# lambdaclass/lambda_elliptic_curves

Hardware: AMD Instinct MI355X
Metric: NTT elems/sec (Stark252 radix-2, 2^24, forward, bit-exact vs CPU: see 'bit_exact') [+ MSM G1 point-adds/sec under 'msm'] (higher is better)
Workload: dtype u32x8 (256-bit Montgomery, 32-bit limbs)

## Files before the change

### lambda_elliptic_curves_amd/csrc/field.cuh

```cuda
#pragma once
#include <stdint.h>

#if defined(__HIPCC__)
#include <hip/hip_runtime.h>
#define LW_HD __host__ __device__ __forceinline__
#else
#define LW_HD inline
#endif

namespace lw {

struct Stark252 {
    static constexpr int N = 8;
    static constexpr bool LAZY = true;
    static constexpr uint32_t INV = 0xffffffffu;
    static constexpr uint32_t TWO_ADICITY = 192;
    LW_HD static constexpr uint32_t p(int i) {
        constexpr uint32_t t[N] = {0x00000001u, 0x00000000u, 0x00000000u, 0x00000000u, 0x00000000u, 0x00000000u, 0x00000011u, 0x08000000u};
        return t[i];
    }
    LW_HD static constexpr uint32_t one(int i) {
        constexpr uint32_t t[N] = {0xffffffe1u, 0xffffffffu, 0xffffffffu, 0xffffffffu, 0xffffffffu, 0xffffffffu, 0xfffffdf0u, 0x07ffffffu};
        return t[i];
    }
    LW_HD static constexpr uint32_t r2(int i) {
        constexpr uint32_t t[N] = {0x7e000401u, 0xfffffd73u, 0x330fffffu, 0x00000001u, 0xff6f8000u, 0xffffffffu, 0x5e008810u, 0x07ffd4abu};
        return t[i];
    }
    LW_HD static constexpr uint32_t root(int i) {
        constexpr uint32_t t[N] = {0x42f8ef94u, 0x6070024fu, 0xe11a6161u, 0xad187148u, 0x9c8b0fa5u, 0x3f046451u, 0x87529cfau, 0x005282dbu};
        return t[i];
    }
};
struct Fr381 {
    static constexpr int N = 8;
    static constexpr bool LAZY = false;
    static constexpr uint32_t INV = 0xffffffffu;
    static constexpr uint32_t TWO_ADICITY = 32;
    LW_HD static constexpr uint32_t p(int i) {
        constexpr uint32_t t[N] = {0x00000001u, 0xffffffffu, 0xfffe5bfeu, 0x53bda402u, 0x09a1d805u, 0x3339d808u, 0x299d7d48u, 0x73eda753u};
        return t[i];
    }
    LW_HD static constexpr uint32_t one(int i) {
        constexpr uint32_t t[N] = {0xfffffffeu, 0x00000001u, 0x00034802u, 0x5884b7fau, 0xecbc4ff5u, 0x998c4fefu, 0xacc5056fu, 0x1824b159u};
        return t[i];
    }
    LW_HD static constexpr uint32_t r2(int i) {
        constexpr uint32_t t[N] = {0xf3f29c6du, 0xc999e990u, 0x87925c23u, 0x2b6cedcbu, 0x7254398fu, 0x05d31496u, 0x9f59ff11u, 0x0748d9d9u};
        return t[i];
    }
    LW_HD static constexpr uint32_t root(int i) {
        constexpr uint32_t t[N] = {0xbb30bbb7u, 0x54cc39d9u, 0xfa78eb2bu, 0xc5e433d6u, 0x349d9b3cu, 0x84dd396cu, 0xa08a499du, 0x2ab00961u};
        return t[i];
    }
};
struct Fp381 {
    static constexpr int N = 12;
    static constexpr uint32_t INV = 0xfffcfffdu;
    LW_HD static constexpr uint32_t p(int i) {
        constexpr uint32_t t[N] = {0xffffaaabu, 0xb9feffffu, 0xb153ffffu, 0x1eabfffeu, 0xf6b0f624u, 0x6730d2a0u, 0xf38512bfu, 0x64774b84u, 0x434bacd7u, 0x4b1ba7b6u, 0x397fe69au, 0x1a0111eau};
        return t[i];
    }
    LW_HD static constexpr uint32_t one(int i) {
        constexpr uint32_t t[N] = {0x0002fffdu, 0x76090000u, 0xc40c0002u, 0xebf4000bu, 0x53c758bau, 0x5f489857u, 0x70525745u, 0x77ce5853u, 0xa256ec6du, 0x5c071a97u, 0xfa80e493u, 0x15f65ec3u};
        return t[i];
    }
    LW_HD static constexpr uint32_t r2(int i) {
        constexpr uint32_t t[N] = {0x1c341746u, 0xf4df1f34u, 0x09d104f1u, 0x0a76e6a6u, 0x4c95b6d5u, 0x8de5476cu, 0x939d83c0u, 0x67eb88a9u, 0xb519952du, 0x9a793e85u, 0x92cae3aau, 0x11988fe5u};
        return t[i];
    }
};
struct Fp254 {
    static constexpr int N = 8;
    static constexpr uint32_t INV = 0xe4866389u;
    LW_HD static constexpr uint32_t p(int i) {
        constexpr uint32_t t[N] = {0xd87cfd47u, 0x3c208c16u, 0x6871ca8du, 0x97816a91u, 0x8181585du, 0xb85045b6u, 0xe131a029u, 0x30644e72u};
        return t[i];
    }
    LW_HD static constexpr uint32_t one(int i) {
        constexpr uint32_t t[N] = {0xc58f0d9du, 0xd35d438du, 0xf5c70b3du, 0x0a78eb28u, 0x7879462cu, 0x666ea36fu, 0x9a07df2fu, 0x0e0a77c1u};
        return t[i];
    }
    LW_HD static constexpr uint32_t r2(int i) {
        constexpr uint32_t t[N] = {0x538afa89u, 0xf32cfc5bu, 0xd44501fbu, 0xb5e71911u, 0x0a417ff6u, 0x47ab1effu, 0xcab8351fu, 0x06d89f71u};
        return t[i];
    }
};

struct Fr254 {
    static constexpr int N = 8;
    static constexpr uint32_t INV = 0xefffffffu;
    static constexpr bool LAZY = false;
    LW_HD static constexpr uint32_t p(int i) {
        constexpr uint32_t t[N] = {0xf0000001u, 0x43e1f593u, 0x79b97091u, 0x2833e848u, 0x8181585du, 0xb85045b6u, 0xe131a029u, 0x30644e72u};
        return t[i];
    }
    LW_HD static constexpr uint32_t one(int i) {
        constexpr uint32_t t[N] = {0x4ffffffbu, 0xac96341cu, 0x9f60cd29u, 0x36fc7695u, 0x7879462eu, 0x666ea36fu, 0x9a07df2fu, 0x0e0a77c1u};
        return t[i];
    }
    LW_HD static constexpr uint32_t r2(int i) {
        constexpr uint32_t t[N] = {0xae216da7u, 0x1bb8e645u, 0xe35c59e3u, 0x53fe3ab1u, 0x53bb8085u, 0x8c49833du, 0x7f4e44a5u, 0x0216d0b1u};
        return t[i];
    }
};

template <class F>
struct Fe {
    static constexpr int N = F::N;
    uint32_t v[F::N];

    LW_HD static Fe zero() {
        Fe r;
#pragma unroll
        for (int i = 0; i < N; i++) r.v[i] = 0;
        return r;
    }
    LW_HD static Fe one() {
        Fe r;
#pragma unroll
        for (int i = 0; i < N; i++) r.v[i] = F::one(i);
        return r;
    }
    LW_HD static Fe r2() {
        Fe r;
#pragma unroll
        for (int i = 0; i < N; i++) r.v[i] = F::r2(i);
        return r;
    }
    LW_HD bool is_zero() const {
        uint32_t o = 0;
#pragma unroll
        for (int i = 0; i < N; i++) o |= v[i];
        return o == 0;
    }
    LW_HD bool operator==(const Fe &b) const {
        uint32_t o = 0;
#pragma unroll
        for (int i = 0; i < N; i++) o |= v[i] ^ b.v[i];
        return o == 0;
    }
    LW_HD bool operator!=(const Fe &b) const { return !(*this == b); }
};

#if defined(__HIP_DEVICE_COMPILE__)
__device__ __forceinline__ uint32_t lw_k(uint32_t x) {
    asm("" : "+s"(x));
    return x;
}
#else
inline uint32_t lw_k(uint32_t x) { return x; }
#endif
#if defined(__clang__)
#define LW_ADDC(a, b, c) __builtin_addc((a), (b), (c), &(c))
#define LW_SUBC(a, b, c) __builtin_subc((a), (b), (c), &(c))
#else
static inline uint32_t lw_addc_portable(uint32_t a, uint32_t b, unsigned &c) {
    const uint64_t t = (uint64_t)a + b + c;
    c = (unsigned)(t >> 32);
    return (uint32_t)t;
}
static inline uint32_t lw_subc_portable(uint32_t a, uint32_t b, unsigned &c) {
    const uint64_t t = (uint64_t)a - b - c;
    c = (unsigned)((t >> 32) & 1);
    return (uint32_t)t;
}
#define LW_ADDC(a, b, c) lw_addc_portable((a), (b), (c))
#define LW_SUBC(a, b, c) lw_subc_portable((a), (b), (c))
#endif
template <int N>
LW_HD uint32_t limbs_add(uint32_t (&r)[N], const uint32_t (&a)[N], const uint32_t (&b)[N]) {
    unsigned c = 0;
#pragma unroll
    for (int i = 0; i < N; i++) r[i] = LW_ADDC(a[i], b[i], c);
    return c;
}
template <int N>
LW_HD uint32_t limbs_sub(uint32_t (&r)[N], const uint32_t (&a)[N], const uint32_t (&b)[N]) {
    unsigned c = 0;
#pragma unroll
    for (int i = 0; i < N; i++) r[i] = LW_SUBC(a[i], b[i], c);
    return c;
}
template <class F, int LOGK>
LW_HD constexpr uint32_t kp_limb(int i) {
    if (LOGK == 0) return F::p(i);
    return (F::p(i) << LOGK) | (i > 0 ? (F::p(i - 1) >> (32 - LOGK)) : 0u);
}
template <class F, int LOGK>
LW_HD void limbs_kp(uint32_t (&k)[F::N]) {
#pragma unroll
    for (int i = 0; i < F::N; i++) k[i] = lw_k(kp_limb<F, LOGK>(i));
}
template <class F>
LW_HD void limbs_p_masked(uint32_t (&k)[F::N], uint32_t mask) {
#pragma unroll
    for (int i = 0; i < F::N; i++) k[i] = F::p(i) == 0 ? lw_k(0u) : (lw_k(F::p(i)) & mask);
}

template <class F>
LW_HD Fe<F> reduce_once(const Fe<F> &a) {
    constexpr int N = F::N;
    uint32_t pk[N];
    limbs_kp<F, 0>(pk);
    Fe<F> d;
    const uint32_t borrow = limbs_sub<N>(d.v, a.v, pk);
    Fe<F> r;
#pragma unroll
    for (int i = 0; i < N; i++) r.v[i] = borrow ? a.v[i] : d.v[i];
    return r;
}

template <class F>
LW_HD Fe<F> fe_add(const Fe<F> &a, const Fe<F> &b) {
    Fe<F> s;
    limbs_add<F::N>(s.v, a.v, b.v);
    return reduce_once<F>(s);
}

template <class F>
LW_HD Fe<F> fe_sub(const Fe<F> &a, const Fe<F> &b) {
    constexpr int N = F::N;
    Fe<F> d;
    const uint32_t borrow = limbs_sub<N>(d.v, a.v, b.v);
    uint32_t pm[N];
    limbs_p_masked<F>(pm, 0u - borrow);
    Fe<F> r;
    limbs_add<N>(r.v, d.v, pm);
    return r;
}

template <class F>
LW_HD Fe<F> fe_neg(const Fe<F> &a) {
    constexpr int N = F::N;
    uint32_t nz = 0;
#pragma unroll
    for (int i = 0; i < N; i++) nz |= a.v[i];
    uint32_t pk[N];
    limbs_kp<F, 0>(pk);
    Fe<F> r;
    limbs_sub<N>(r.v, pk, a.v);
#pragma unroll
    for (int i = 0; i < N; i++) r.v[i] = nz ? r.v[i] : 0u;
    return r;
}

template <class F>
LW_HD Fe<F> fe_dbl(const Fe<F> &a) { return fe_add<F>(a, a); }

template <class F>
LW_HD Fe<F> fe_mul_portable(const Fe<F> &a, const Fe<F> &b) {
    constexpr int N = F::N;
    uint32_t t[N];
#pragma unroll
    for (int i = 0; i < N; i++) t[i] = 0;
#pragma unroll
    for (int i = 0; i < N; i++) {
        uint64_t c = 0;
#pragma unroll
        for (int j = 0; j < N; j++) {
            c += (uint64_t)a.v[j] * b.v[i] + t[j];
            t[j] = (uint32_t)c;
            c >>= 32;
        }
        uint32_t tN = (uint32_t)c;
        uint32_t m = t[0] * F::INV;
        c = ((uint64_t)m * F::p(0) + t[0]) >> 32;
#pragma unroll
        for (int j = 1; j < N; j++) {
            c += (uint64_t)m * F::p(j) + t[j];
            t[j - 1] = (uint32_t)c;
            c >>= 32;
        }
        c += tN;
        t[N - 1] = (uint32_t)c;
    }
    Fe<F> r;
#pragma unroll
    for (int i = 0; i < N; i++) r.v[i] = t[i];
    return reduce_once<F>(r);
}

#if !defined(__HIP_DEVICE_COMPILE__) && defined(__SIZEOF_INT128__)
#define LW_HOST_MUL64 1
template <class F>
inline Fe<F> fe_mul_host64(const Fe<F> &a, const Fe<F> &b) {
    constexpr int N = F::N, M = N / 2;
    static_assert(N % 2 == 0, "even number of 32-bit limbs");
    typedef unsigned __int128 u128;
    uint64_t A[M], B[M], P[M], t[M + 2];
    for (int i = 0; i < M; i++) {
        A[i] = (uint64_t)a.v[2 * i] | ((uint64_t)a.v[2 * i + 1] << 32);
        B[i] = (uint64_t)b.v[2 * i] | ((uint64_t)b.v[2 * i + 1] << 32);
        P[i] = (uint64_t)F::p(2 * i) | ((uint64_t)F::p(2 * i + 1) << 32);
    }
    for (int i = 0; i < M + 2; i++) t[i] = 0;
    uint64_t z = (uint64_t)(0u - F::INV);
    z *= 2 - P[0] * z;
    const uint64_t inv = 0 - z;
    for (int i = 0; i < M; i++) {
        u128 c = 0;
        for (int j = 0; j < M; j++) {
            c += (u128)A[j] * B[i] + t[j];
            t[j] = (uint64_t)c;
            c >>= 64;
        }
        c += t[M];
        t[M] = (uint64_t)c;
        t[M + 1] = (uint64_t)(c >> 64);
        const uint64_t m = t[0] * inv;
        c = ((u128)m * P[0] + t[0]) >> 64;
        for (int j = 1; j < M; j++) {
            c += (u128)m * P[j] + t[j];
            t[j - 1] = (uint64_t)c;
            c >>= 64;
        }
        c += t[M];
        t[M - 1] = (uint64_t)c;
        t[M] = t[M + 1] + (uint64_t)(c >> 64);
    }
    Fe<F> r;
    for (int i = 0; i < M; i++) {
        r.v[2 * i] = (uint32_t)t[i];
        r.v[2 * i + 1] = (uint32_t)(t[i] >> 32);
    }
    return reduce_once<F>(r);
}
#endif

#if defined(__HIP_DEVICE_COMPILE__)
#define LW_MAC_V(A, B) "v_mad_u64_u32 %0, vcc, " A ", " B ", %0\n\tv_addc_co_u32_e32 %1, vcc, 0, %1, vcc\n\t"

__device__ __forceinline__ void mac96_x1(uint64_t &lo, uint32_t &hi, uint32_t a0, uint32_t b0) {
    asm(LW_MAC_V("%2", "%3") : "+v"(lo), "+v"(hi) : "v"(a0), "v"(b0) : "vcc");
}
__device__ __forceinline__ void mac96_x2(uint64_t &lo, uint32_t &hi, uint32_t a0, uint32_t b0, uint32_t a1, uint32_t b1) {
    asm(LW_MAC_V("%2", "%3") LW_MAC_V("%4", "%5") : "+v"(lo), "+v"(hi) : "v"(a0), "v"(b0), "v"(a1), "v"(b1) : "vcc");
}
__device__ __forceinline__ void mac96_x4(uint64_t &lo, uint32_t &hi, uint32_t a0, uint32_t b0, uint32_t a1, uint32_t b1,
                                         uint32_t a2, uint32_t b2, uint32_t a3, uint32_t b3) {
    asm(LW_MAC_V("%2", "%3") LW_MAC_V("%4", "%5") LW_MAC_V("%6", "%7") LW_MAC_V("%8", "%9")
        : "+v"(lo), "+v"(hi)
        : "v"(a0), "v"(b0), "v"(a1), "v"(b1), "v"(a2), "v"(b2), "v"(a3), "v"(b3)
        : "vcc");
}
#define LW_MAC_FIRST(A, B, INIT) "v_mad_u64_u32 %0, vcc, " A ", " B ", " INIT "\n\tv_addc_co_u32_e64 %1, vcc, 0, 0, vcc\n\t"
template <uint32_t C>
__device__ __forceinline__ void mac96_c1(uint64_t &lo, uint32_t &hi, uint32_t m0) {
    if constexpr (C == 0) {
    } else if constexpr (C <= 64) {
        asm(LW_MAC_V("%2", "%3") : "+v"(lo), "+v"(hi) : "v"(m0), "n"(C) : "vcc");
    } else {
        asm(LW_MAC_V("%2", "%3") : "+v"(lo), "+v"(hi) : "v"(m0), "s"(C) : "vcc");
    }
}
template <uint32_t C0, uint32_t C1, uint32_t C2, uint32_t C3>
__device__ __forceinline__ void mac96_s4(uint64_t &lo, uint32_t &hi, uint32_t m0, uint32_t m1, uint32_t m2, uint32_t m3) {
    asm(LW_MAC_V("%2", "%3") LW_MAC_V("%4", "%5") LW_MAC_V("%6", "%7") LW_MAC_V("%8", "%9")
        : "+v"(lo), "+v"(hi)
        : "v"(m0), "s"(C0), "v"(m1), "s"(C1), "v"(m2), "s"(C2), "v"(m3), "s"(C3)
        : "vcc");
}

template <class F, int K, int I, int IEND>
__device__ __forceinline__ void col_ab(uint64_t &lo, uint32_t &hi, const Fe<F> &a, const Fe<F> &b) {
    if constexpr (I + 4 <= IEND) {
        mac96_x4(lo, hi, a.v[I], b.v[K - I], a.v[I + 1], b.v[K - I - 1], a.v[I + 2], b.v[K - I - 2], a.v[I + 3], b.v[K - I - 3]);
        col_ab<F, K, I + 4, IEND>(lo, hi, a, b);
    } else if constexpr (I + 2 <= IEND) {
        mac96_x2(lo, hi, a.v[I], b.v[K - I], a.v[I + 1], b.v[K - I - 1]);
        col_ab<F, K, I + 2, IEND>(lo, hi, a, b);
    } else if constexpr (I + 1 <= IEND) {
        mac96_x1(lo, hi, a.v[I], b.v[K - I]);
    }
}
template <uint32_t C>
constexpr bool lw_is_literal() { return C > 64; }
template <class F, int K, int I, int IEND>
__device__ __forceinline__ void col_mp(uint64_t &lo, uint32_t &hi, const uint32_t (&m)[F::N]) {
    if constexpr (I + 4 <= IEND) {
        if constexpr (lw_is_literal<F::p(K - I)>() && lw_is_literal<F::p(K - I - 1)>() && lw_is_literal<F::p(K - I - 2)>() &&
                      lw_is_literal<F::p(K - I - 3)>()) {
            mac96_s4<F::p(K - I), F::p(K - I - 1), F::p(K - I - 2), F::p(K - I - 3)>(lo, hi, m[I], m[I + 1], m[I + 2], m[I + 3]);
            col_mp<F, K, I + 4, IEND>(lo, hi, m);
        } else {
            mac96_c1<F::p(K - I)>(lo, hi, m[I]);
            col_mp<F, K, I + 1, IEND>(lo, hi, m);
        }
    } else if constexpr (I + 1 <= IEND) {
        mac96_c1<F::p(K - I)>(lo, hi, m[I]);
        col_mp<F, K, I + 1, IEND>(lo, hi, m);
    }
}
template <class F>
struct lw_fused_columns {
    static constexpr bool value = false;
};
template <class F, int K, bool A_LT_P>
struct FusedCol;
#include "mac_chains.inc"

template <class F, int LO, int HI>
constexpr bool lw_all_literal() {
    for (int i = LO; i < HI; i++)
        if (F::p(i) <= 64) return false;
    return true;
}

template <class F, int P, int K>
__device__ __forceinline__ void fips_col(uint64_t init, const Fe<F> *const (&a)[P], const Fe<F> *const (&b)[P], uint32_t (&m)[F::N],
                                         uint32_t (&t)[F::N]) {
    constexpr int N = F::N;
    if constexpr (K == 2 * N - 1) {
        t[N - 1] = (uint32_t)init;
    } else {
        uint64_t lo;
        uint32_t hi;
        if constexpr (K < N) {
            col_ab_first_dispatch<F, K, 0, K + 1>(lo, hi, init, *a[0], *b[0]);
            if constexpr (P > 1) col_ab<F, K, 0, K + 1>(lo, hi, *a[1], *b[1]);
            if constexpr (P > 2) col_ab<F, K, 0, K + 1>(lo, hi, *a[2], *b[2]);
            if constexpr (P > 3) col_ab<F, K, 0, K + 1>(lo, hi, *a[3], *b[3]);
            if constexpr (K >= 1 && lw_all_literal<F, 1, K + 1>()) col_mp_dispatch<F, K, 0, K>(lo, hi, m);
            else col_mp<F, K, 0, K>(lo, hi, m);
            uint32_t mk;
            if constexpr (F::INV == 0xffffffffu) mk = 0u - (uint32_t)lo;
            else mk = (uint32_t)lo * F::INV;
            m[K] = mk;
            mac96_c1<F::p(0)>(lo, hi, mk);
        } else {
            col_ab_first_dispatch<F, K, K - N + 1, 2 * N - 1 - K>(lo, hi, init, *a[0], *b[0]);
            if constexpr (P > 1) col_ab<F, K, K - N + 1, N>(lo, hi, *a[1], *b[1]);
            if constexpr (P > 2) col_ab<F, K, K - N + 1, N>(lo, hi, *a[2], *b[2]);
            if constexpr (P > 3) col_ab<F, K, K - N + 1, N>(lo, hi, *a[3], *b[3]);
            if constexpr (lw_all_literal<F, K - N + 1, N>()) col_mp_dispatch<F, K, K - N + 1, 2 * N - 1 - K>(lo, hi, m);
            else col_mp<F, K, K - N + 1, N>(lo, hi, m);
            t[K - N] = (uint32_t)lo;
        }
        fips_col<F, P, K + 1>((lo >> 32) | ((uint64_t)hi << 32), a, b, m, t);
    }
}
__device__ __forceinline__ void lw_redc_unit(uint32_t &m, uint32_t &mid, uint32_t &top, uint32_t t, uint32_t w1, uint32_t w2) {
    asm("v_sub_co_u32_e32 %0, vcc, 0, %3\n\t"
        "v_addc_co_u32_e32 %1, vcc, 0, %4, vcc\n\t"
        "v_addc_co_u32_e32 %2, vcc, 0, %5, vcc"
        : "=&v"(m), "=&v"(mid), "=v"(top)
        : "v"(t), "v"(w1), "v"(w2)
        : "vcc");
}
__device__ __forceinline__ void lw_redc_unit0(uint32_t &m, uint32_t &mid, uint32_t &top, uint32_t t, uint32_t w1) {
    asm("v_sub_co_u32_e32 %0, vcc, 0, %3\n\t"
        "v_addc_co_u32_e32 %1, vcc, 0, %4, vcc\n\t"
        "v_addc_co_u32_e64 %2, vcc, 0, 0, vcc"
        : "=&v"(m), "=&v"(mid), "=v"(top)
        : "v"(t), "v"(w1)
        : "vcc");
}
template <class F, int K, bool A_LT_P>
__device__ __forceinline__ void fips_fused(uint64_t init, const Fe<F> &a, const Fe<F> &b, uint32_t (&m)[F::N], uint32_t (&t)[F::N]) {
    constexpr int N = F::N;
    static_assert(F::p(0) == 1u && F::INV == 0xffffffffu, "fused columns need a unit low limb of the modulus");
    if constexpr (K == 2 * N - 1) {
        t[N - 1] = (uint32_t)init;
    } else {
        uint64_t lo;
        uint32_t hi;
        FusedCol<F, K, A_LT_P>::run(lo, hi, init, a, b, m);
        if constexpr (K < N) {
            uint32_t mid, top;
            if constexpr (K == 0) lw_redc_unit0(m[0], mid, top, (uint32_t)lo, (uint32_t)(lo >> 32));
            else lw_redc_unit(m[K], mid, top, (uint32_t)lo, (uint32_t)(lo >> 32), hi);
            fips_fused<F, K + 1, A_LT_P>(((uint64_t)top << 32) | mid, a, b, m, t);
        } else {
            t[K - N] = (uint32_t)lo;
            fips_fused<F, K + 1, A_LT_P>((lo >> 32) | ((uint64_t)hi << 32), a, b, m, t);
        }
    }
}
template <class F, bool A_LT_P = false>
__device__ __forceinline__ void fips_product(const Fe<F> &a, const Fe<F> &b, uint32_t (&t)[F::N]) {
    uint32_t m[F::N];
    if constexpr (lw_fused_columns<F>::value) {
        fips_fused<F, 0, A_LT_P>(0ull, a, b, m, t);
    } else {
        const Fe<F> *const pa[1] = {&a}, *const pb[1] = {&b};
        fips_col<F, 1, 0>(0ull, pa, pb, m, t);
    }
}
template <class F>
__device__ __forceinline__ Fe<F> fe_mul_gfx9(const Fe<F> &a, const Fe<F> &b) {
    constexpr int N = F::N;
    uint32_t t[N];
    fips_product<F>(a, b, t);
    Fe<F> r;
#pragma unroll
    for (int i = 0; i < N; i++) r.v[i] = t[i];
    return reduce_once<F>(r);
}
#endif

template <class F>
LW_HD Fe<F> fe_mul(const Fe<F> &a, const Fe<F> &b) {
#if defined(__HIP_DEVICE_COMPILE__)
    return fe_mul_gfx9<F>(a, b);
#elif defined(LW_HOST_MUL64)
    return fe_mul_host64<F>(a, b);
#else
    return fe_mul_portable<F>(a, b);
#endif
}

template <class F>
LW_HD Fe<F> fe_sqr(const Fe<F> &a) { return fe_mul<F>(a, a); }

template <class F>
LW_HD Fe<F> fe_neg_raw(const Fe<F> &a) {
    uint32_t pk[F::N];
    limbs_kp<F, 0>(pk);
    Fe<F> r;
    limbs_sub<F::N>(r.v, pk, a.v);
    return r;
}
template <class F>
LW_HD Fe<F> fe_neg_raw_2p(const Fe<F> &a) {
    uint32_t pk[F::N];
    limbs_kp<F, 1>(pk);
    Fe<F> r;
    limbs_sub<F::N>(r.v, pk, a.v);
    return r;
}
template <class F, int P, int KSUM = P>
LW_HD Fe<F> fe_dot(const Fe<F> *const (&a)[P], const Fe<F> *const (&b)[P]) {
    static_assert(P >= 1 && P <= 4, "fe_dot: 1..4 products");
    static_assert(KSUM >= P, "fe_dot: KSUM counts every product at least once");
    static_assert((uint64_t)KSUM * ((uint64_t)F::p(F::N - 1) + 1) <= (1ull << 32), "fe_dot: sum of products would exceed 2p after reduction");
#if defined(__HIP_DEVICE_COMPILE__)
    constexpr int N = F::N;
    uint32_t m[N], t[N];
    fips_col<F, P, 0>(0ull, a, b, m, t);
    Fe<F> r;
#pragma unroll
    for (int i = 0; i < N; i++) r.v[i] = t[i];
    return reduce_once<F>(r);
#else
    static_assert(KSUM == P, "fe_dot: unreduced operands are a device-code feature");
    Fe<F> acc = fe_mul<F>(reduce_once<F>(*a[0]), *b[0]);
    for (int q = 1; q < P; q++) acc = fe_add<F>(acc, fe_mul<F>(reduce_once<F>(*a[q]), *b[q]));
    return acc;
#endif
}

template <class F, int LOGK>
LW_HD Fe<F> fe_cond_sub_kp(const Fe<F> &a) {
    constexpr int N = F::N;
    uint32_t kp[N];
    limbs_kp<F, LOGK>(kp);
    Fe<F> d;
    const uint32_t borrow = limbs_sub<N>(d.v, a.v, kp);
    Fe<F> r;
#pragma unroll
    for (int i = 0; i < N; i++) r.v[i] = borrow ? a.v[i] : d.v[i];
    return r;
}
LW_HD Fe<Stark252> fe_reduce_full(const Fe<Stark252> &x) {
    const uint32_t q = x.v[7] >> 27;
    const uint32_t z = lw_k(0u);
    const uint32_t sub[8] = {q, z, z, z, z, z, 17u * q, q << 27};
    Fe<Stark252> d;
    const uint32_t borrow = limbs_sub<8>(d.v, x.v, sub);
    uint32_t pm[8];
    limbs_p_masked<Stark252>(pm, 0u - borrow);
    Fe<Stark252> r;
    limbs_add<8>(r.v, d.v, pm);
    return r;
}
template <class F>
LW_HD Fe<F> fe_reduce_full(const Fe<F> &x) { return reduce_once<F>(x); }

template <class F>
LW_HD Fe<F> fe_add_raw(const Fe<F> &a, const Fe<F> &b) {
    Fe<F> s;
    limbs_add<F::N>(s.v, a.v, b.v);
    return s;
}
template <class F>
LW_HD Fe<F> fe_add2p_sub_raw(const Fe<F> &a, const Fe<F> &b) {
    constexpr int N = F::N;
    uint32_t kp[N];
    limbs_kp<F, 1>(kp);
    Fe<F> d, r;
    limbs_sub<N>(d.v, a.v, b.v);
    limbs_add<N>(r.v, d.v, kp);
    return r;
}
template <class F>
LW_HD Fe<F> fe_mul_lazy(const Fe<F> &a, const Fe<F> &b) {
#if defined(__HIP_DEVICE_COMPILE__)
    constexpr int N = F::N;
    uint32_t t[N];
    fips_product<F, true>(a, b, t);
    Fe<F> r;
#pragma unroll
    for (int i = 0; i < N; i++) r.v[i] = t[i];
    return r;
#else
    return fe_mul_portable<F>(a, b);
#endif
}

template <class F>
LW_HD Fe<F> fe_pow_u64(Fe<F> base, uint64_t e) {
    Fe<F> r = Fe<F>::one();
    while (e) {
        if (e & 1) r = fe_mul<F>(r, base);
        base = fe_sqr<F>(base);
        e >>= 1;
    }
    return r;
}

template <class F>
LW_HD Fe<F> fe_inv(const Fe<F> &a) {
    constexpr int N = F::N;
    uint32_t e[N];
    uint64_t borrow = 2;
#pragma unroll
    for (int i = 0; i < N; i++) {
        uint64_t t = (uint64_t)F::p(i) - borrow;
        e[i] = (uint32_t)t;
        borrow = (t >> 32) & 1;
    }
    Fe<F> r = Fe<F>::one();
    for (int i = N - 1; i >= 0; i--) {
        for (int bit = 31; bit >= 0; bit--) {
            r = fe_sqr<F>(r);
            if ((e[i] >> bit) & 1) r = fe_mul<F>(r, a);
        }
    }
    return r;
}

template <class F>
LW_HD constexpr int fe_modulus_bits() {
    int top = 0;
    for (int b = 0; b < 32; b++)
        if ((F::p(F::N - 1) >> b) & 1u) top = b + 1;
    return 32 * (F::N - 1) + top;
}
template <int N>
LW_HD uint32_t bingcd_update_ab(uint32_t (&x)[N], uint32_t (&y)[N], int32_t f, int32_t g, int32_t h, int32_t k) {
    int64_t cx = 0, cy = 0;
    uint32_t wx[N + 1], wy[N + 1];
#pragma unroll
    for (int i = 0; i < N; i++) {
        const int64_t zx = (int64_t)x[i] * f + (int64_t)y[i] * g + cx;
        const int64_t zy = (int64_t)x[i] * h + (int64_t)y[i] * k + cy;
        wx[i] = (uint32_t)zx;
        wy[i] = (uint32_t)zy;
        cx = zx >> 32;
        cy = zy >> 32;
    }
    wx[N] = (uint32_t)cx;
    wy[N] = (uint32_t)cy;
    const uint32_t nx = (uint32_t)((uint64_t)cx >> 63), ny = (uint32_t)((uint64_t)cy >> 63);
    uint32_t carx = nx, cary = ny;
#pragma unroll
    for (int i = 0; i < N; i++) {
        uint32_t rx = (wx[i] >> 30) | (wx[i + 1] << 2), ry = (wy[i] >> 30) | (wy[i + 1] << 2);
        rx ^= 0u - nx;
        ry ^= 0u - ny;
        const uint32_t sx = rx + carx, sy = ry + cary;
        carx = sx < rx ? 1u : 0u;
        cary = sy < ry ? 1u : 0u;
        x[i] = sx;
        y[i] = sy;
    }
    return nx | (ny << 1);
}
template <class F>
LW_HD void bingcd_update_uv(uint32_t (&u)[F::N], uint32_t (&v)[F::N], int32_t f, int32_t g, int32_t h, int32_t k) {
    constexpr int N = F::N;
    const uint32_t fu = ((uint32_t)(u[0] * (uint32_t)f + v[0] * (uint32_t)g) * F::INV) & 0x3fffffffu;
    const uint32_t fv = ((uint32_t)(u[0] * (uint32_t)h + v[0] * (uint32_t)k) * F::INV) & 0x3fffffffu;
    int64_t cu = 0, cv = 0;
    uint32_t wu[N + 1], wv[N + 1];
#pragma unroll
    for (int i = 0; i < N; i++) {
        const int64_t zu = (int64_t)u[i] * f + (int64_t)v[i] * g + (int64_t)((uint64_t)F::p(i) * fu) + cu;
        const int64_t zv = (int64_t)u[i] * h + (int64_t)v[i] * k + (int64_t)((uint64_t)F::p(i) * fv) + cv;
        wu[i] = (uint32_t)zu;
        wv[i] = (uint32_t)zv;
        cu = zu >> 32;
        cv = zv >> 32;
    }
    wu[N] = (uint32_t)cu;
    wv[N] = (uint32_t)cv;
    const uint32_t nu = (uint32_t)((uint64_t)cu >> 63), nv = (uint32_t)((uint64_t)cv >> 63);
    uint32_t ru[N], rv[N];
#pragma unroll
    for (int i = 0; i < N; i++) {
        ru[i] = (wu[i] >> 30) | (wu[i + 1] << 2);
        rv[i] = (wv[i] >> 30) | (wv[i + 1] << 2);
    }
    uint32_t pk[N], du[N], dv[N], su[N], sv[N];
#pragma unroll
    for (int i = 0; i < N; i++) pk[i] = F::p(i);
    const uint32_t bu = limbs_sub<N>(du, ru, pk), bv = limbs_sub<N>(dv, rv, pk);
    limbs_add<N>(su, ru, pk);
    limbs_add<N>(sv, rv, pk);
#pragma unroll
    for (int i = 0; i < N; i++) {
        u[i] = nu ? su[i] : (bu ? ru[i] : du[i]);
        v[i] = nv ? sv[i] : (bv ? rv[i] : dv[i]);
    }
}
template <class F>
LW_HD Fe<F> fe_inv_int_bingcd(const Fe<F> &y) {
    constexpr int N = F::N;
    constexpr int ROUNDS = (2 * fe_modulus_bits<F>()) / 29 + 2;
    uint32_t a[N], b[N], u[N], v[N];
#pragma unroll
    for (int i = 0; i < N; i++) {
        a[i] = y.v[i];
        b[i] = F::p(i);
        u[i] = i == 0 ? 1u : 0u;
        v[i] = 0u;
    }
#pragma nounroll
    for (int round = 0; round < ROUNDS; round++) {
        uint32_t a0 = 0, a1 = 0, b0 = 0, b1 = 0, c0 = 0xffffffffu, c1 = 0xffffffffu;
#pragma unroll
        for (int j = N - 1; j >= 0; j--) {
            const uint32_t aw = a[j], bw = b[j];
            a0 ^= (a0 ^ aw) & c0;
            a1 ^= (a1 ^ aw) & c1;
            b0 ^= (b0 ^ bw) & c0;
            b1 ^= (b1 ^ bw) & c1;
            c1 = c0;
            c0 &= ((aw | bw) == 0u) ? 0xffffffffu : 0u;
        }
        a1 |= a0 & c1;
        a0 &= ~c1;
        b1 |= b0 & c1;
        b0 &= ~c1;
        uint64_t a_hi = ((uint64_t)a0 << 32) | a1, b_hi = ((uint64_t)b0 << 32) | b1;
        uint32_t a_lo = a[0], b_lo = b[0];
        int32_t pa = 1, pb = 0, qa = 0, qb = 1;
#pragma unroll 2
        for (int i = 0; i < 30; i++) {
            const uint32_t r = a_hi > b_hi ? 1u : 0u;
            const uint32_t oa = (a_lo >> i) & 1u, ob = (b_lo >> i) & 1u;
            const uint32_t cAB = oa & ob & r, cBA = oa & ob & (r ^ 1u), cA = cAB | (oa ^ 1u);
            const uint32_t mAB = 0u - cAB, mBA = 0u - cBA, mA = 0u - cA;
            a_lo -= b_lo & mAB;
            a_hi -= b_hi & (uint64_t)(int64_t)(int32_t)mAB;
            pa -= qa & (int32_t)mAB;
            pb -= qb & (int32_t)mAB;
            b_lo -= a_lo & mBA;
            b_hi -= a_hi & (uint64_t)(int64_t)(int32_t)mBA;
            qa -= pa & (int32_t)mBA;
            qb -= pb & (int32_t)mBA;
            a_lo += a_lo & ~mA;
            pa += pa & (int32_t)~mA;
            pb += pb & (int32_t)~mA;
            a_hi = cA ? (a_hi >> 1) : a_hi;
            b_lo += b_lo & mA;
            qa += qa & (int32_t)mA;
            qb += qb & (int32_t)mA;
            b_hi = cA ? b_hi : (b_hi >> 1);
        }
        const uint32_t neg = bingcd_update_ab<N>(a, b, pa, pb, qa, qb);
        if (neg & 1u) { pa = -pa; pb = -pb; }
        if (neg & 2u) { qa = -qa; qb = -qb; }
        bingcd_update_uv<F>(u, v, pa, pb, qa, qb);
    }
    Fe<F> r;
    const bool zero = y.is_zero();
#pragma unroll
    for (int i = 0; i < N; i++) r.v[i] = zero ? 0u : (u[i] | v[i]);
    return r;
}
template <class F>
LW_HD Fe<F> fe_inv_fast(const Fe<F> &a) {
    const Fe<F> r3 = fe_mul<F>(Fe<F>::r2(), Fe<F>::r2());
    return fe_mul<F>(fe_inv_int_bingcd<F>(a), r3);
}

template <class F>
LW_HD Fe<F> fe_to_mont(const Fe<F> &a) { return fe_mul<F>(a, Fe<F>::r2()); }
template <class F>
LW_HD Fe<F> fe_from_mont(const Fe<F> &a) {
    Fe<F> o = Fe<F>::zero();
    o.v[0] = 1;
    return fe_mul<F>(a, o);
}
template <class F>
LW_HD Fe<F> fe_from_u64(uint64_t x) {
    Fe<F> o = Fe<F>::zero();
    o.v[0] = (uint32_t)x;
    o.v[1] = (uint32_t)(x >> 32);
    return fe_to_mont<F>(o);
}

template <class F>
LW_HD constexpr int mem_index(int k) { return 2 * (F::N / 2 - 1 - k / 2) + (k & 1); }

template <class F>
LW_HD Fe<F> fe_load(const void *ptr) {
    constexpr int N = F::N;
    const uint4 *q = reinterpret_cast<const uint4 *>(ptr);
    uint32_t m[N];
#pragma unroll
    for (int i = 0; i < N / 4; i++) {
        uint4 x = q[i];
        m[4 * i + 0] = x.x; m[4 * i + 1] = x.y; m[4 * i + 2] = x.z; m[4 * i + 3] = x.w;
    }
    Fe<F> r;
#pragma unroll
    for (int k = 0; k < N; k++) r.v[k] = m[mem_index<F>(k)];
    return r;
}
template <class F>
LW_HD void fe_store(void *ptr, const Fe<F> &a) {
    constexpr int N = F::N;
    uint32_t m[N];
#pragma unroll
    for (int k = 0; k < N; k++) m[mem_index<F>(k)] = a.v[k];
    uint4 *q = reinterpret_cast<uint4 *>(ptr);
#pragma unroll
    for (int i = 0; i < N / 4; i++) q[i] = make_uint4(m[4 * i], m[4 * i + 1], m[4 * i + 2], m[4 * i + 3]);
}

struct BabyBear {
    static constexpr uint32_t P = 2013265921u;
    static constexpr uint32_t MU = 0x88000001u;
    static constexpr uint32_t R2 = 0x45dddde3u;
    static constexpr uint32_t ONE = 0x0ffffffeu;
    static constexpr uint32_t TWO_ADICITY = 24;
    static constexpr uint32_t ROOT = 21;
};

LW_HD uint32_t bb_reduce(uint64_t x) {
    const uint32_t m = (uint32_t)x * (0u - BabyBear::MU);
    const uint32_t r = (uint32_t)((x + (uint64_t)m * BabyBear::P) >> 32);
    const uint32_t d = r - BabyBear::P;
    return d < r ? d : r;
}
LW_HD uint32_t bb_mul(uint32_t a, uint32_t b) { return bb_reduce((uint64_t)a * b); }
LW_HD uint32_t bb_add(uint32_t a, uint32_t b) {
    const uint32_t s = a + b, d = s - BabyBear::P;
    return d < s ? d : s;
}
LW_HD uint32_t bb_sub(uint32_t a, uint32_t b) {
    const uint32_t d = a - b, e = d + BabyBear::P;
    return e < d ? e : d;
}
LW_HD uint32_t bb_pow(uint32_t a, uint64_t e) {
    uint32_t r = BabyBear::ONE;
    while (e) {
        if (e & 1) r = bb_mul(r, a);
        a = bb_mul(a, a);
        e >>= 1;
    }
    return r;
}
LW_HD uint32_t bb_inv(uint32_t a) { return bb_pow(a, (uint64_t)BabyBear::P - 2); }
LW_HD uint32_t bb_from_r64(uint64_t w) { return bb_reduce(w); }
LW_HD uint64_t bb_to_r64(uint32_t v) { return (uint64_t)bb_mul(v, BabyBear::R2); }

}
```

### lambda_elliptic_curves_amd/csrc/mac_chains.inc

```

template <class F, int K, int I>
__device__ __forceinline__ void col_ab_first_n1(uint64_t &lo, uint32_t &hi, uint64_t init, const Fe<F> &a, const Fe<F> &b) {
    asm(LW_MAC_FIRST("%3", "%4", "%2")
        : "=v"(lo), "=v"(hi)
        : "v"(init), "v"(a.v[I + 0]), "v"(b.v[K - I - 0])
        : "vcc");
}

template <class F, int K, int I>
__device__ __forceinline__ void col_ab_first_n2(uint64_t &lo, uint32_t &hi, uint64_t init, const Fe<F> &a, const Fe<F> &b) {
    asm(LW_MAC_FIRST("%3", "%4", "%2") LW_MAC_V("%5", "%6")
        : "=&v"(lo), "=&v"(hi)
        : "v"(init), "v"(a.v[I + 0]), "v"(b.v[K - I - 0]), "v"(a.v[I + 1]), "v"(b.v[K - I - 1])
        : "vcc");
}

template <class F, int K, int I>
__device__ __forceinline__ void col_ab_first_n3(uint64_t &lo, uint32_t &hi, uint64_t init, const Fe<F> &a, const Fe<F> &b) {
    asm(LW_MAC_FIRST("%3", "%4", "%2") LW_MAC_V("%5", "%6") LW_MAC_V("%7", "%8")
        : "=&v"(lo), "=&v"(hi)
        : "v"(init), "v"(a.v[I + 0]), "v"(b.v[K - I - 0]), "v"(a.v[I + 1]), "v"(b.v[K - I - 1]), "v"(a.v[I + 2]), "v"(b.v[K - I - 2])
        : "vcc");
}

template <class F, int K, int I>
__device__ __forceinline__ void col_ab_first_n4(uint64_t &lo, uint32_t &hi, uint64_t init, const Fe<F> &a, const Fe<F> &b) {
    asm(LW_MAC_FIRST("%3", "%4", "%2") LW_MAC_V("%5", "%6") LW_MAC_V("%7", "%8") LW_MAC_V("%9", "%10")
        : "=&v"(lo), "=&v"(hi)
        : "v"(init), "v"(a.v[I + 0]), "v"(b.v[K - I - 0]), "v"(a.v[I + 1]), "v"(b.v[K - I - 1]), "v"(a.v[I + 2]), "v"(b.v[K - I - 2]), "v"(a.v[I + 3]), "v"(b.v[K - I - 3])
        : "vcc");
}

template <class F, int K, int I>
__device__ __forceinline__ void col_ab_first_n5(uint64_t &lo, uint32_t &hi, uint64_t init, const Fe<F> &a, const Fe<F> &b) {
    asm(LW_MAC_FIRST("%3", "%4", "%2") LW_MAC_V("%5", "%6") LW_MAC_V("%7", "%8") LW_MAC_V("%9", "%10") LW_MAC_V("%11", "%12")
        : "=&v"(lo), "=&v"(hi)
        : "v"(init), "v"(a.v[I + 0]), "v"(b.v[K - I - 0]), "v"(a.v[I + 1]), "v"(b.v[K - I - 1]), "v"(a.v[I + 2]), "v"(b.v[K - I - 2]), "v"(a.v[I + 3]), "v"(b.v[K - I - 3]), "v"(a.v[I + 4]), "v"(b.v[K - I - 4])
        : "vcc");
}

template <class F, int K, int I>
__device__ __forceinline__ void col_ab_first_n6(uint64_t &lo, uint32_t &hi, uint64_t init, const Fe<F> &a, const Fe<F> &b) {
    asm(LW_MAC_FIRST("%3", "%4", "%2") LW_MAC_V("%5", "%6") LW_MAC_V("%7", "%8") LW_MAC_V("%9", "%10") LW_MAC_V("%11", "%12") LW_MAC_V("%13", "%14")
        : "=&v"(lo), "=&v"(hi)
        : "v"(init), "v"(a.v[I + 0]), "v"(b.v[K - I - 0]), "v"(a.v[I + 1]), "v"(b.v[K - I - 1]), "v"(a.v[I + 2]), "v"(b.v[K - I - 2]), "v"(a.v[I + 3]), "v"(b.v[K - I - 3]), "v"(a.v[I + 4]), "v"(b.v[K - I - 4]), "v"(a.v[I + 5]), "v"(b.v[K - I - 5])
        : "vcc");
}

template <class F, int K, int I>
__device__ __forceinline__ void col_ab_first_n7(uint64_t &lo, uint32_t &hi, uint64_t init, const Fe<F> &a, const Fe<F> &b) {
    asm(LW_MAC_FIRST("%3", "%4", "%2") LW_MAC_V("%5", "%6") LW_MAC_V("%7", "%8") LW_MAC_V("%9", "%10") LW_MAC_V("%11", "%12") LW_MAC_V("%13", "%14") LW_MAC_V("%15", "%16")
        : "=&v"(lo), "=&v"(hi)
        : "v"(init), "v"(a.v[I + 0]), "v"(b.v[K - I - 0]), "v"(a.v[I + 1]), "v"(b.v[K - I - 1]), "v"(a.v[I + 2]), "v"(b.v[K - I - 2]), "v"(a.v[I + 3]), "v"(b.v[K - I - 3]), "v"(a.v[I + 4]), "v"(b.v[K - I - 4]), "v"(a.v[I + 5]), "v"(b.v[K - I - 5]), "v"(a.v[I + 6]), "v"(b.v[K - I - 6])
        : "vcc");
}

template <class F, int K, int I>
__device__ __forceinline__ void col_ab_first_n8(uint64_t &lo, uint32_t &hi, uint64_t init, const Fe<F> &a, const Fe<F> &b) {
    asm(LW_MAC_FIRST("%3", "%4", "%2") LW_MAC_V("%5", "%6") LW_MAC_V("%7", "%8") LW_MAC_V("%9", "%10") LW_MAC_V("%11", "%12") LW_MAC_V("%13", "%14") LW_MAC_V("%15", "%16") LW_MAC_V("%17", "%18")
        : "=&v"(lo), "=&v"(hi)
        : "v"(init), "v"(a.v[I + 0]), "v"(b.v[K - I - 0]), "v"(a.v[I + 1]), "v"(b.v[K - I - 1]), "v"(a.v[I + 2]), "v"(b.v[K - I - 2]), "v"(a.v[I + 3]), "v"(b.v[K - I - 3]), "v"(a.v[I + 4]), "v"(b.v[K - I - 4]), "v"(a.v[I + 5]), "v"(b.v[K - I - 5]), "v"(a.v[I + 6]), "v"(b.v[K - I - 6]), "v"(a.v[I + 7]), "v"(b.v[K - I - 7])
        : "vcc");
}

template <class F, int K, int I>
__device__ __forceinline__ void col_ab_first_n9(uint64_t &lo, uint32_t &hi, uint64_t init, const Fe<F> &a, const Fe<F> &b) {
    asm(LW_MAC_FIRST("%3", "%4", "%2") LW_MAC_V("%5", "%6") LW_MAC_V("%7", "%8") LW_MAC_V("%9", "%10") LW_MAC_V("%11", "%12") LW_MAC_V("%13", "%14") LW_MAC_V("%15", "%16") LW_MAC_V("%17", "%18") LW_MAC_V("%19", "%20")
        : "=&v"(lo), "=&v"(hi)
        : "v"(init), "v"(a.v[I + 0]), "v"(b.v[K - I - 0]), "v"(a.v[I + 1]), "v"(b.v[K - I - 1]), "v"(a.v[I + 2]), "v"(b.v[K - I - 2]), "v"(a.v[I + 3]), "v"(b.v[K - I - 3]), "v"(a.v[I + 4]), "v"(b.v[K - I - 4]), "v"(a.v[I + 5]), "v"(b.v[K - I - 5]), "v"(a.v[I + 6]), "v"(b.v[K - I - 6]), "v"(a.v[I + 7]), "v"(b.v[K - I - 7]), "v"(a.v[I + 8]), "v"(b.v[K - I - 8])
        : "vcc");
}

template <class F, int K, int I>
__device__ __forceinline__ void col_ab_first_n10(uint64_t &lo, uint32_t &hi, uint64_t init, const Fe<F> &a, const Fe<F> &b) {
    asm(LW_MAC_FIRST("%3", "%4", "%2") LW_MAC_V("%5", "%6") LW_MAC_V("%7", "%8") LW_MAC_V("%9", "%10") LW_MAC_V("%11", "%12") LW_MAC_V("%13", "%14") LW_MAC_V("%15", "%16") LW_MAC_V("%17", "%18") LW_MAC_V("%19", "%20") LW_MAC_V("%21", "%22")
        : "=&v"(lo), "=&v"(hi)
        : "v"(init), "v"(a.v[I + 0]), "v"(b.v[K - I - 0]), "v"(a.v[I + 1]), "v"(b.v[K - I - 1]), "v"(a.v[I + 2]), "v"(b.v[K - I - 2]), "v"(a.v[I + 3]), "v"(b.v[K - I - 3]), "v"(a.v[I + 4]), "v"(b.v[K - I - 4]), "v"(a.v[I + 5]), "v"(b.v[K - I - 5]), "v"(a.v[I + 6]), "v"(b.v[K - I - 6]), "v"(a.v[I + 7]), "v"(b.v[K - I - 7]), "v"(a.v[I + 8]), "v"(b.v[K - I - 8]), "v"(a.v[I + 9]), "v"(b.v[K - I - 9])
        : "vcc");
}

template <class F, int K, int I>
__device__ __forceinline__ void col_ab_first_n11(uint64_t &lo, uint32_t &hi, uint64_t init, const Fe<F> &a, const Fe<F> &b) {
    asm(LW_MAC_FIRST("%3", "%4", "%2") LW_MAC_V("%5", "%6") LW_MAC_V("%7", "%8") LW_MAC_V("%9", "%10") LW_MAC_V("%11", "%12") LW_MAC_V("%13", "%14") LW_MAC_V("%15", "%16") LW_MAC_V("%17", "%18") LW_MAC_V("%19", "%20") LW_MAC_V("%21", "%22") LW_MAC_V("%23", "%24")
        : "=&v"(lo), "=&v"(hi)
        : "v"(init), "v"(a.v[I + 0]), "v"(b.v[K - I - 0]), "v"(a.v[I + 1]), "v"(b.v[K - I - 1]), "v"(a.v[I + 2]), "v"(b.v[K - I - 2]), "v"(a.v[I + 3]), "v"(b.v[K - I - 3]), "v"(a.v[I + 4]), "v"(b.v[K - I - 4]), "v"(a.v[I + 5]), "v"(b.v[K - I - 5]), "v"(a.v[I + 6]), "v"(b.v[K - I - 6]), "v"(a.v[I + 7]), "v"(b.v[K - I - 7]), "v"(a.v[I + 8]), "v"(b.v[K - I - 8]), "v"(a.v[I + 9]), "v"(b.v[K - I - 9]), "v"(a.v[I + 10]), "v"(b.v[K - I - 10])
        : "vcc");
}

template <class F, int K, int I>
__device__ __forceinline__ void col_ab_first_n12(uint64_t &lo, uint32_t &hi, uint64_t init, const Fe<F> &a, const Fe<F> &b) {
    asm(LW_MAC_FIRST("%3", "%4", "%2") LW_MAC_V("%5", "%6") LW_MAC_V("%7", "%8") LW_MAC_V("%9", "%10") LW_MAC_V("%11", "%12") LW_MAC_V("%13", "%14") LW_MAC_V("%15", "%16") LW_MAC_V("%17", "%18") LW_MAC_V("%19", "%20") LW_MAC_V("%21", "%22") LW_MAC_V("%23", "%24") LW_MAC_V("%25", "%26")
        : "=&v"(lo), "=&v"(hi)
        : "v"(init), "v"(a.v[I + 0]), "v"(b.v[K - I - 0]), "v"(a.v[I + 1]), "v"(b.v[K - I - 1]), "v"(a.v[I + 2]), "v"(b.v[K - I - 2]), "v"(a.v[I + 3]), "v"(b.v[K - I - 3]), "v"(a.v[I + 4]), "v"(b.v[K - I - 4]), "v"(a.v[I + 5]), "v"(b.v[K - I - 5]), "v"(a.v[I + 6]), "v"(b.v[K - I - 6]), "v"(a.v[I + 7]), "v"(b.v[K - I - 7]), "v"(a.v[I + 8]), "v"(b.v[K - I - 8]), "v"(a.v[I + 9]), "v"(b.v[K - I - 9]), "v"(a.v[I + 10]), "v"(b.v[K - I - 10]), "v"(a.v[I + 11]), "v"(b.v[K - I - 11])
        : "vcc");
}

template <class F, int K, int I>
__device__ __forceinline__ void col_mp_n1(uint64_t &lo, uint32_t &hi, const uint32_t (&m)[F::N]) {
    asm(LW_MAC_V("%2", "%3")
        : "+v"(lo), "+v"(hi)
        : "v"(m[I + 0]), "s"(F::p(K - I - 0))
        : "vcc");
}

template <class F, int K, int I>
__device__ __forceinline__ void col_mp_n2(uint64_t &lo, uint32_t &hi, const uint32_t (&m)[F::N]) {
    asm(LW_MAC_V("%2", "%3") LW_MAC_V("%4", "%5")
        : "+v"(lo), "+v"(hi)
        : "v"(m[I + 0]), "s"(F::p(K - I - 0)), "v"(m[I + 1]), "s"(F::p(K - I - 1))
        : "vcc");
}

template <class F, int K, int I>
__device__ __forceinline__ void col_mp_n3(uint64_t &lo, uint32_t &hi, const uint32_t (&m)[F::N]) {
    asm(LW_MAC_V("%2", "%3") LW_MAC_V("%4", "%5") LW_MAC_V("%6", "%7")
        : "+v"(lo), "+v"(hi)
        : "v"(m[I + 0]), "s"(F::p(K - I - 0)), "v"(m[I + 1]), "s"(F::p(K - I - 1)), "v"(m[I + 2]), "s"(F::p(K - I - 2))
        : "vcc");
}

template <class F, int K, int I>
__device__ __forceinline__ void col_mp_n4(uint64_t &lo, uint32_t &hi, const uint32_t (&m)[F::N]) {
    asm(LW_MAC_V("%2", "%3") LW_MAC_V("%4", "%5") LW_MAC_V("%6", "%7") LW_MAC_V("%8", "%9")
        : "+v"(lo), "+v"(hi)
        : "v"(m[I + 0]), "s"(F::p(K - I - 0)), "v"(m[I + 1]), "s"(F::p(K - I - 1)), "v"(m[I + 2]), "s"(F::p(K - I - 2)), "v"(m[I + 3]), "s"(F::p(K - I - 3))
        : "vcc");
}

template <class F, int K, int I>
__device__ __forceinline__ void col_mp_n5(uint64_t &lo, uint32_t &hi, const uint32_t (&m)[F::N]) {
    asm(LW_MAC_V("%2", "%3") LW_MAC_V("%4", "%5") LW_MAC_V("%6", "%7") LW_MAC_V("%8", "%9") LW_MAC_V("%10", "%11")
        : "+v"(lo), "+v"(hi)
        : "v"(m[I + 0]), "s"(F::p(K - I - 0)), "v"(m[I + 1]), "s"(F::p(K - I - 1)), "v"(m[I + 2]), "s"(F::p(K - I - 2)), "v"(m[I + 3]), "s"(F::p(K - I - 3)), "v"(m[I + 4]), "s"(F::p(K - I - 4))
        : "vcc");
}

template <class F, int K, int I>
__device__ __forceinline__ void col_mp_n6(uint64_t &lo, uint32_t &hi, const uint32_t (&m)[F::N]) {
    asm(LW_MAC_V("%2", "%3") LW_MAC_V("%4", "%5") LW_MAC_V("%6", "%7") LW_MAC_V("%8", "%9") LW_MAC_V("%10", "%11") LW_MAC_V("%12", "%13")
        : "+v"(lo), "+v"(hi)
        : "v"(m[I + 0]), "s"(F::p(K - I - 0)), "v"(m[I + 1]), "s"(F::p(K - I - 1)), "v"(m[I + 2]), "s"(F::p(K - I - 2)), "v"(m[I + 3]), "s"(F::p(K - I - 3)), "v"(m[I + 4]), "s"(F::p(K - I - 4)), "v"(m[I + 5]), "s"(F::p(K - I - 5))
        : "vcc");
}

template <class F, int K, int I>
__device__ __forceinline__ void col_mp_n7(uint64_t &lo, uint32_t &hi, const uint32_t (&m)[F::N]) {
    asm(LW_MAC_V("%2", "%3") LW_MAC_V("%4", "%5") LW_MAC_V("%6", "%7") LW_MAC_V("%8", "%9") LW_MAC_V("%10", "%11") LW_MAC_V("%12", "%13") LW_MAC_V("%14", "%15")
        : "+v"(lo), "+v"(hi)
        : "v"(m[I + 0]), "s"(F::p(K - I - 0)), "v"(m[I + 1]), "s"(F::p(K - I - 1)), "v"(m[I + 2]), "s"(F::p(K - I - 2)), "v"(m[I + 3]), "s"(F::p(K - I - 3)), "v"(m[I + 4]), "s"(F::p(K - I - 4)), "v"(m[I + 5]), "s"(F::p(K - I - 5)), "v"(m[I + 6]), "s"(F::p(K - I - 6))
        : "vcc");
}

template <class F, int K, int I>
__device__ __forceinline__ void col_mp_n8(uint64_t &lo, uint32_t &hi, const uint32_t (&m)[F::N]) {
    asm(LW_MAC_V("%2", "%3") LW_MAC_V("%4", "%5") LW_MAC_V("%6", "%7") LW_MAC_V("%8", "%9") LW_MAC_V("%10", "%11") LW_MAC_V("%12", "%13") LW_MAC_V("%14", "%15") LW_MAC_V("%16", "%17")
        : "+v"(lo), "+v"(hi)
        : "v"(m[I + 0]), "s"(F::p(K - I - 0)), "v"(m[I + 1]), "s"(F::p(K - I - 1)), "v"(m[I + 2]), "s"(F::p(K - I - 2)), "v"(m[I + 3]), "s"(F::p(K - I - 3)), "v"(m[I + 4]), "s"(F::p(K - I - 4)), "v"(m[I + 5]), "s"(F::p(K - I - 5)), "v"(m[I + 6]), "s"(F::p(K - I - 6)), "v"(m[I + 7]), "s"(F::p(K - I - 7))
        : "vcc");
}

template <class F, int K, int I>
__device__ __forceinline__ void col_mp_n9(uint64_t &lo, uint32_t &hi, const uint32_t (&m)[F::N]) {
    asm(LW_MAC_V("%2", "%3") LW_MAC_V("%4", "%5") LW_MAC_V("%6", "%7") LW_MAC_V("%8", "%9") LW_MAC_V("%10", "%11") LW_MAC_V("%12", "%13") LW_MAC_V("%14", "%15") LW_MAC_V("%16", "%17") LW_MAC_V("%18", "%19")
        : "+v"(lo), "+v"(hi)
        : "v"(m[I + 0]), "s"(F::p(K - I - 0)), "v"(m[I + 1]), "s"(F::p(K - I - 1)), "v"(m[I + 2]), "s"(F::p(K - I - 2)), "v"(m[I + 3]), "s"(F::p(K - I - 3)), "v"(m[I + 4]), "s"(F::p(K - I - 4)), "v"(m[I + 5]), "s"(F::p(K - I - 5)), "v"(m[I + 6]), "s"(F::p(K - I - 6)), "v"(m[I + 7]), "s"(F::p(K - I - 7)), "v"(m[I + 8]), "s"(F::p(K - I - 8))
        : "vcc");
}

template <class F, int K, int I>
__device__ __forceinline__ void col_mp_n10(uint64_t &lo, uint32_t &hi, const uint32_t (&m)[F::N]) {
    asm(LW_MAC_V("%2", "%3") LW_MAC_V("%4", "%5") LW_MAC_V("%6", "%7") LW_MAC_V("%8", "%9") LW_MAC_V("%10", "%11") LW_MAC_V("%12", "%13") LW_MAC_V("%14", "%15") LW_MAC_V("%16", "%17") LW_MAC_V("%18", "%19") LW_MAC_V("%20", "%21")
        : "+v"(lo), "+v"(hi)
        : "v"(m[I + 0]), "s"(F::p(K - I - 0)), "v"(m[I + 1]), "s"(F::p(K - I - 1)), "v"(m[I + 2]), "s"(F::p(K - I - 2)), "v"(m[I + 3]), "s"(F::p(K - I - 3)), "v"(m[I + 4]), "s"(F::p(K - I - 4)), "v"(m[I + 5]), "s"(F::p(K - I - 5)), "v"(m[I + 6]), "s"(F::p(K - I - 6)), "v"(m[I + 7]), "s"(F::p(K - I - 7)), "v"(m[I + 8]), "s"(F::p(K - I - 8)), "v"(m[I + 9]), "s"(F::p(K - I - 9))
        : "vcc");
}

template <class F, int K, int I>
__device__ __forceinline__ void col_mp_n11(uint64_t &lo, uint32_t &hi, const uint32_t (&m)[F::N]) {
    asm(LW_MAC_V("%2", "%3") LW_MAC_V("%4", "%5") LW_MAC_V("%6", "%7") LW_MAC_V("%8", "%9") LW_MAC_V("%10", "%11") LW_MAC_V("%12", "%13") LW_MAC_V("%14", "%15") LW_MAC_V("%16", "%17") LW_MAC_V("%18", "%19") LW_MAC_V("%20", "%21") LW_MAC_V("%22", "%23")
        : "+v"(lo), "+v"(hi)
        : "v"(m[I + 0]), "s"(F::p(K - I - 0)), "v"(m[I + 1]), "s"(F::p(K - I - 1)), "v"(m[I + 2]), "s"(F::p(K - I - 2)), "v"(m[I + 3]), "s"(F::p(K - I - 3)), "v"(m[I + 4]), "s"(F::p(K - I - 4)), "v"(m[I + 5]), "s"(F::p(K - I - 5)), "v"(m[I + 6]), "s"(F::p(K - I - 6)), "v"(m[I + 7]), "s"(F::p(K - I - 7)), "v"(m[I + 8]), "s"(F::p(K - I - 8)), "v"(m[I + 9]), "s"(F::p(K - I - 9)), "v"(m[I + 10]), "s"(F::p(K - I - 10))
        : "vcc");
}

template <class F, int K, int I, int CNT>
__device__ __forceinline__ void col_ab_first_dispatch(uint64_t &lo, uint32_t &hi, uint64_t init, const Fe<F> &a, const Fe<F> &b) {
    if constexpr (CNT == 1) col_ab_first_n1<F, K, I>(lo, hi, init, a, b);
    else if constexpr (CNT == 2) col_ab_first_n2<F, K, I>(lo, hi, init, a, b);
    else if constexpr (CNT == 3) col_ab_first_n3<F, K, I>(lo, hi, init, a, b);
    else if constexpr (CNT == 4) col_ab_first_n4<F, K, I>(lo, hi, init, a, b);
    else if constexpr (CNT == 5) col_ab_first_n5<F, K, I>(lo, hi, init, a, b);
    else if constexpr (CNT == 6) col_ab_first_n6<F, K, I>(lo, hi, init, a, b);
    else if constexpr (CNT == 7) col_ab_first_n7<F, K, I>(lo, hi, init, a, b);
    else if constexpr (CNT == 8) col_ab_first_n8<F, K, I>(lo, hi, init, a, b);
    else if constexpr (CNT == 9) col_ab_first_n9<F, K, I>(lo, hi, init, a, b);
    else if constexpr (CNT == 10) col_ab_first_n10<F, K, I>(lo, hi, init, a, b);
    else if constexpr (CNT == 11) col_ab_first_n11<F, K, I>(lo, hi, init, a, b);
    else if constexpr (CNT == 12) col_ab_first_n12<F, K, I>(lo, hi, init, a, b);
    else static_assert(CNT >= 1 && CNT <= 12, "unsupported MAC count");
}

template <class F, int K, int I, int CNT>
__device__ __forceinline__ void col_mp_dispatch(uint64_t &lo, uint32_t &hi, const uint32_t (&m)[F::N]) {
    if constexpr (CNT == 1) col_mp_n1<F, K, I>(lo, hi, m);
    else if constexpr (CNT == 2) col_mp_n2<F, K, I>(lo, hi, m);
    else if constexpr (CNT == 3) col_mp_n3<F, K, I>(lo, hi, m);
    else if constexpr (CNT == 4) col_mp_n4<F, K, I>(lo, hi, m);
    else if constexpr (CNT == 5) col_mp_n5<F, K, I>(lo, hi, m);
    else if constexpr (CNT == 6) col_mp_n6<F, K, I>(lo, hi, m);
    else if constexpr (CNT == 7) col_mp_n7<F, K, I>(lo, hi, m);
    else if constexpr (CNT == 8) col_mp_n8<F, K, I>(lo, hi, m);
    else if constexpr (CNT == 9) col_mp_n9<F, K, I>(lo, hi, m);
    else if constexpr (CNT == 10) col_mp_n10<F, K, I>(lo, hi, m);
    else if constexpr (CNT == 11) col_mp_n11<F, K, I>(lo, hi, m);
    else static_assert(CNT >= 1 && CNT <= 11, "unsupported MAC count");
}

static_assert(Stark252::N == 8 && Stark252::p(0) == 0x00000001u && Stark252::p(1) == 0x00000000u && Stark252::p(2) == 0x00000000u && Stark252::p(3) == 0x00000000u && Stark252::p(4) == 0x00000000u && Stark252::p(5) == 0x00000000u && Stark252::p(6) == 0x00000011u && Stark252::p(7) == 0x08000000u, "modulus changed: rerun tools/gen_mac_chains.py");
template <>
struct lw_fused_columns<Stark252> {
    static constexpr bool value = true;
};

template <>
struct FusedCol<Stark252, 0, false> {
    __device__ static __forceinline__ void run(uint64_t &lo, uint32_t &hi, uint64_t init, const Fe<Stark252> &a, const Fe<Stark252> &b, const uint32_t (&m)[8]) {
        asm("v_mad_u64_u32 %0, vcc, %1, %2, 0\n\t"
            : "=v"(lo)
            : "v"(a.v[0]), "v"(b.v[0])
            : "vcc");
        hi = 0;
    }
};

template <>
struct FusedCol<Stark252, 1, false> {
    __device__ static __forceinline__ void run(uint64_t &lo, uint32_t &hi, uint64_t init, const Fe<Stark252> &a, const Fe<Stark252> &b, const uint32_t (&m)[8]) {
        asm("v_mad_u64_u32 %0, vcc, %3, %4, %2\n\t"
            "v_mad_u64_u32 %0, vcc, %5, %6, %0\n\t"
            "v_addc_co_u32_e64 %1, vcc, 0, 0, vcc\n\t"
            : "=&v"(lo), "=&v"(hi)
            : "v"(init), "v"(a.v[0]), "v"(b.v[1]), "v"(a.v[1]), "v"(b.v[0])
            : "vcc");
    }
};

template <>
struct FusedCol<Stark252, 2, false> {
    __device__ static __forceinline__ void run(uint64_t &lo, uint32_t &hi, uint64_t init, const Fe<Stark252> &a, const Fe<Stark252> &b, const uint32_t (&m)[8]) {
        asm("v_mad_u64_u32 %0, vcc, %3, %4, %2\n\t"
            "v_mad_u64_u32 %0, vcc, %5, %6, %0\n\t"
            "v_addc_co_u32_e64 %1, vcc, 0, 0, vcc\n\t"
            "v_mad_u64_u32 %0, vcc, %7, %8, %0\n\t"
            "v_addc_co_u32_e32 %1, vcc, 0, %1, vcc\n\t"
            : "=&v"(lo), "=&v"(hi)
            : "v"(init), "v"(a.v[0]), "v"(b.v[2]), "v"(a.v[1]), "v"(b.v[1]), "v"(a.v[2]), "v"(b.v[0])
            : "vcc");
    }
};

template <>
struct FusedCol<Stark252, 3, false> {
    __device__ static __forceinline__ void run(uint64_t &lo, uint32_t &hi, uint64_t init, const Fe<Stark252> &a, const Fe<Stark252> &b, const uint32_t (&m)[8]) {
        asm("v_mad_u64_u32 %0, vcc, %3, %4, %2\n\t"
            "v_addc_co_u32_e64 %1, vcc, 0, 0, vcc\n\t"
            "v_mad_u64_u32 %0, vcc, %5, %6, %0\n\t"
            "v_addc_co_u32_e32 %1, vcc, 0, %1, vcc\n\t"
            "v_mad_u64_u32 %0, vcc, %7, %8, %0\n\t"
            "v_addc_co_u32_e32 %1, vcc, 0, %1, vcc\n\t"
            "v_mad_u64_u32 %0, vcc, %9, %10, %0\n\t"
            "v_addc_co_u32_e32 %1, vcc, 0, %1, vcc\n\t"
            : "=&v"(lo), "=&v"(hi)
            : "v"(init), "v"(a.v[0]), "v"(b.v[3]), "v"(a.v[1]), "v"(b.v[2]), "v"(a.v[2]), "v"(b.v[1]), "v"(a.v[3]), "v"(b.v[0])
            : "vcc");
    }
};

template <>
struct FusedCol<Stark252, 4, false> {
    __device__ static __forceinline__ void run(uint64_t &lo, uint32_t &hi, uint64_t init, const Fe<Stark252> &a, const Fe<Stark252> &b, const uint32_t (&m)[8]) {
        asm("v_mad_u64_u32 %0, vcc, %3, %4, %2\n\t"
            "v_addc_co_u32_e64 %1, vcc, 0, 0, vcc\n\t"
            "v_mad_u64_u32 %0, vcc, %5, %6, %0\n\t"
            "v_addc_co_u32_e32 %1, vcc, 0, %1, vcc\n\t"
            "v_mad_u64_u32 %0, vcc, %7, %8, %0\n\t"
            "v_addc_co_u32_e32 %1, vcc, 0, %1, vcc\n\t"
            "v_mad_u64_u32 %0, vcc, %9, %10, %0\n\t"
            "v_addc_co_u32_e32 %1, vcc, 0, %1, vcc\n\t"
            "v_mad_u64_u32 %0, vcc, %11, %12, %0\n\t"
            "v_addc_co_u32_e32 %1, vcc, 0, %1, vcc\n\t"
            : "=&v"(lo), "=&v"(hi)
            : "v"(init), "v"(a.v[0]), "v"(b.v[4]), "v"(a.v[1]), "v"(b.v[3]), "v"(a.v[2]), "v"(b.v[2]), "v"(a.v[3]), "v"(b.v[1]), "v"(a.v[4]), "v"(b.v[0])
            : "vcc");
    }
};

template <>
struct FusedCol<Stark252, 5, false> {
    __device__ static __forceinline__ void run(uint64_t &lo, uint32_t &hi, uint64_t init, const Fe<Stark252> &a, const Fe<Stark252> &b, const uint32_t (&m)[8]) {
        asm("v_mad_u64_u32 %0, vcc, %3, %4, %2\n\t"
            "v_addc_co_u32_e64 %1, vcc, 0, 0, vcc\n\t"
            "v_mad_u64_u32 %0, vcc, %5, %6, %0\n\t"
            "v_addc_co_u32_e32 %1, vcc, 0, %1, vcc\n\t"
            "v_mad_u64_u32 %0, vcc, %7, %8, %0\n\t"
            "v_addc_co_u32_e32 %1, vcc, 0, %1, vcc\n\t"
            "v_mad_u64_u32 %0, vcc, %9, %10, %0\n\t"
            "v_addc_co_u32_e32 %1, vcc, 0, %1, vcc\n\t"
            "v_mad_u64_u32 %0, vcc, %11, %12, %0\n\t"
            "v_addc_co_u32_e32 %1, vcc, 0, %1, vcc\n\t"
            "v_mad_u64_u32 %0, vcc, %13, %14, %0\n\t"
            "v_addc_co_u32_e32 %1, vcc, 0, %1, vcc\n\t"
            : "=&v"(lo), "=&v"(hi)
            : "v"(init), "v"(a.v[0]), "v"(b.v[5]), "v"(a.v[1]), "v"(b.v[4]), "v"(a.v[2]), "v"(b.v[3]), "v"(a.v[3]), "v"(b.v[2]), "v"(a.v[4]), "v"(b.v[1]), "v"(a.v[5]), "v"(b.v[0])
            : "vcc");
    }
};

template <>
struct FusedCol<Stark252, 6, false> {
    __device__ static __forceinline__ void run(uint64_t &lo, uint32_t &hi, uint64_t init, const Fe<Stark252> &a, const Fe<Stark252> &b, const uint32_t (&m)[8]) {
        asm("v_mad_u64_u32 %0, vcc, %3, 17, %2\n\t"
            "v_mad_u64_u32 %0, vcc, %4, %5, %0\n\t"
            "v_addc_co_u32_e64 %1, vcc, 0, 0, vcc\n\t"
            "v_mad_u64_u32 %0, vcc, %6, %7, %0\n\t"
            "v_addc_co_u32_e32 %1, vcc, 0, %1, vcc\n\t"
            "v_mad_u64_u32 %0, vcc, %8, %9, %0\n\t"
            "v_addc_co_u32_e32 %1, vcc, 0, %1, vcc\n\t"
            "v_mad_u64_u32 %0, vcc, %10, %11, %0\n\t"
            "v_addc_co_u32_e32 %1, vcc, 0, %1, vcc\n\t"
            "v_mad_u64_u32 %0, vcc, %12, %13, %0\n\t"
            "v_addc_co_u32_e32 %1, vcc, 0, %1, vcc\n\t"
            "v_mad_u64_u32 %0, vcc, %14, %15, %0\n\t"
            "v_addc_co_u32_e32 %1, vcc, 0, %1, vcc\n\t"
            "v_mad_u64_u32 %0, vcc, %16, %17, %0\n\t"
            "v_addc_co_u32_e32 %1, vcc, 0, %1, vcc\n\t"
            : "=&v"(lo), "=&v"(hi)
            : "v"(init), "v"(m[0]), "v"(a.v[0]), "v"(b.v[6]), "v"(a.v[1]), "v"(b.v[5]), "v"(a.v[2]), "v"(b.v[4]), "v"(a.v[3]), "v"(b.v[3]), "v"(a.v[4]), "v"(b.v[2]), "v"(a.v[5]), "v"(b.v[1]), "v"(a.v[6]), "v"(b.v[0])
            : "vcc");
    }
};

template <>
struct FusedCol<Stark252, 7, false> {
    __device__ static __forceinline__ void run(uint64_t &lo, uint32_t &hi, uint64_t init, const Fe<Stark252> &a, const Fe<Stark252> &b, const uint32_t (&m)[8]) {
        asm("v_mad_u64_u32 %0, vcc, %3, %4, %2\n\t"
            "v_mad_u64_u32 %0, vcc, %5, 17, %0\n\t"
            "v_mad_u64_u32 %0, vcc, %6, %7, %0\n\t"
            "v_addc_co_u32_e64 %1, vcc, 0, 0, vcc\n\t"
            "v_mad_u64_u32 %0, vcc, %8, %9, %0\n\t"
            "v_addc_co_u32_e32 %1, vcc, 0, %1, vcc\n\t"
            "v_mad_u64_u32 %0, vcc, %10, %11, %0\n\t"
            "v_addc_co_u32_e32 %1, vcc, 0, %1, vcc\n\t"
            "v_mad_u64_u32 %0, vcc, %12, %13, %0\n\t"
            "v_addc_co_u32_e32 %1, vcc, 0, %1, vcc\n\t"
            "v_mad_u64_u32 %0, vcc, %14, %15, %0\n\t"
            "v_addc_co_u32_e32 %1, vcc, 0, %1, vcc\n\t"
            "v_mad_u64_u32 %0, vcc, %16, %17, %0\n\t"
            "v_addc_co_u32_e32 %1, vcc, 0, %1, vcc\n\t"
            "v_mad_u64_u32 %0, vcc, %18, %19, %0\n\t"
            "v_addc_co_u32_e32 %1, vcc, 0, %1, vcc\n\t"
            "v_mad_u64_u32 %0, vcc, %20, %21, %0\n\t"
            "v_addc_co_u32_e32 %1, vcc, 0, %1, vcc\n\t"
            : "=&v"(lo), "=&v"(hi)
            : "v"(init), "v"(m[0]), "s"(Stark252::p(7)), "v"(m[1]), "v"(a.v[0]), "v"(b.v[7]), "v"(a.v[1]), "v"(b.v[6]), "v"(a.v[2]), "v"(b.v[5]), "v"(a.v[3]), "v"(b.v[4]), "v"(a.v[4]), "v"(b.v[3]), "v"(a.v[5]), "v"(b.v[2]), "v"(a.v[6]), "v"(b.v[1]), "v"(a.v[7]), "v"(b.v[0])
            : "vcc");
    }
};

template <>
struct FusedCol<Stark252, 8, false> {
    __device__ static __forceinline__ void run(uint64_t &lo, uint32_t &hi, uint64_t init, const Fe<Stark252> &a, const Fe<Stark252> &b, const uint32_t (&m)[8]) {
        asm("v_mad_u64_u32 %0, vcc, %3, %4, %2\n\t"
            "v_mad_u64_u32 %0, vcc, %5, 17, %0\n\t"
            "v_mad_u64_u32 %0, vcc, %6, %7, %0\n\t"
            "v_addc_co_u32_e64 %1, vcc, 0, 0, vcc\n\t"
            "v_mad_u64_u32 %0, vcc, %8, %9, %0\n\t"
            "v_addc_co_u32_e32 %1, vcc, 0, %1, vcc\n\t"
            "v_mad_u64_u32 %0, vcc, %10, %11, %0\n\t"
            "v_addc_co_u32_e32 %1, vcc, 0, %1, vcc\n\t"
            "v_mad_u64_u32 %0, vcc, %12, %13, %0\n\t"
            "v_addc_co_u32_e32 %1, vcc, 0, %1, vcc\n\t"
            "v_mad_u64_u32 %0, vcc, %14, %15, %0\n\t"
            "v_addc_co_u32_e32 %1, vcc, 0, %1, vcc\n\t"
            "v_mad_u64_u32 %0, vcc, %16, %17, %0\n\t"
            "v_addc_co_u32_e32 %1, vcc, 0, %1, vcc\n\t"
            "v_mad_u64_u32 %0, vcc, %18, %19, %0\n\t"
            "v_addc_co_u32_e32 %1, vcc, 0, %1, vcc\n\t"
            : "=&v"(lo), "=&v"(hi)
            : "v"(init), "v"(m[1]), "s"(Stark252::p(7)), "v"(m[2]), "v"(a.v[1]), "v"(b.v[7]), "v"(a.v[2]), "v"(b.v[6]), "v"(a.v[3]), "v"(b.v[5]), "v"(a.v[4]), "v"(b.v[4]), "v"(a.v[5]), "v"(b.v[3]), "v"(a.v[6]), "v"(b.v[2]), "v"(a.v[7]), "v"(b.v[1])
            : "vcc");
    }
};

template <>
struct FusedCol<Stark252, 9, false> {
    __device__ static __forceinline__ void run(uint64_t &lo, uint32_t &hi, uint64_t init, const Fe<Stark252> &a, const Fe<Stark252> &b, const uint32_t (&m)[8]) {
        asm("v_mad_u64_u32 %0, vcc, %3, %4, %2\n\t"
            "v_mad_u64_u32 %0, vcc, %5, 17, %0\n\t"
            "v_mad_u64_u32 %0, vcc, %6, %7, %0\n\t"
            "v_addc_co_u32_e64 %1, vcc, 0, 0, vcc\n\t"
            "v_mad_u64_u32 %0, vcc, %8, %9, %0\n\t"
            "v_addc_co_u32_e32 %1, vcc, 0, %1, vcc\n\t"
            "v_mad_u64_u32 %0, vcc, %10, %11, %0\n\t"
            "v_addc_co_u32_e32 %1, vcc, 0, %1, vcc\n\t"
            "v_mad_u64_u32 %0, vcc, %12, %13, %0\n\t"
            "v_addc_co_u32_e32 %1, vcc, 0, %1, vcc\n\t"
            "v_mad_u64_u32 %0, vcc, %14, %15, %0\n\t"
            "v_addc_co_u32_e32 %1, vcc, 0, %1, vcc\n\t"
            "v_mad_u64_u32 %0, vcc, %16, %17, %0\n\t"
            "v_addc_co_u32_e32 %1, vcc, 0, %1, vcc\n\t"
            : "=&v"(lo), "=&v"(hi)
            : "v"(init), "v"(m[2]), "s"(Stark252::p(7)), "v"(m[3]), "v"(a.v[2]), "v"(b.v[7]), "v"(a.v[3]), "v"(b.v[6]), "v"(a.v[4]), "v"(b.v[5]), "v"(a.v[5]), "v"(b.v[4]), "v"(a.v[6]), "v"(b.v[3]), "v"(a.v[7]), "v"(b.v[2])
            : "vcc");
    }
};

template <>
struct FusedCol<Stark252, 10, false> {
    __device__ static __forceinline__ void run(uint64_t &lo, uint32_t &hi, uint64_t init, const Fe<Stark252> &a, const Fe<Stark252> &b, const uint32_t (&m)[8]) {
        asm("v_mad_u64_u32 %0, vcc, %3, %4, %2\n\t"
            "v_mad_u64_u32 %0, vcc, %5, 17, %0\n\t"
            "v_mad_u64_u32 %0, vcc, %6, %7, %0\n\t"
            "v_addc_co_u32_e64 %1, vcc, 0, 0, vcc\n\t"
            "v_mad_u64_u32 %0, vcc, %8, %9, %0\n\t"
            "v_addc_co_u32_e32 %1, vcc, 0, %1, vcc\n\t"
            "v_mad_u64_u32 %0, vcc, %10, %11, %0\n\t"
            "v_addc_co_u32_e32 %1, vcc, 0, %1, vcc\n\t"
            "v_mad_u64_u32 %0, vcc, %12, %13, %0\n\t"
            "v_addc_co_u32_e32 %1, vcc, 0, %1, vcc\n\t"
            "v_mad_u64_u32 %0, vcc, %14, %15, %0\n\t"
            "v_addc_co_u32_e32 %1, vcc, 0, %1, vcc\n\t"
            : "=&v"(lo), "=&v"(hi)
            : "v"(init), "v"(m[3]), "s"(Stark252::p(7)), "v"(m[4]), "v"(a.v[3]), "v"(b.v[7]), "v"(a.v[4]), "v"(b.v[6]), "v"(a.v[5]), "v"(b.v[5]), "v"(a.v[6]), "v"(b.v[4]), "v"(a.v[7]), "v"(b.v[3])
            : "vcc");
    }
};

template <>
struct FusedCol<Stark252, 11, false> {
    __device__ static __forceinline__ void run(uint64_t &lo, uint32_t &hi, uint64_t init, const Fe<Stark252> &a, const Fe<Stark252> &b, const uint32_t (&m)[8]) {
        asm("v_mad_u64_u32 %0, vcc, %3, %4, %2\n\t"
            "v_mad_u64_u32 %0, vcc, %5, 17, %0\n\t"
            "v_mad_u64_u32 %0, vcc, %6, %7, %0\n\t"
            "v_addc_co_u32_e64 %1, vcc, 0, 0, vcc\n\t"
            "v_mad_u64_u32 %0, vcc, %8, %9, %0\n\t"
            "v_addc_co_u32_e32 %1, vcc, 0, %1, vcc\n\t"
            "v_mad_u64_u32 %0, vcc, %10, %11, %0\n\t"
            "v_addc_co_u32_e32 %1, vcc, 0, %1, vcc\n\t"
            "v_mad_u64_u32 %0, vcc, %12, %13, %0\n\t"
            "v_addc_co_u32_e32 %1, vcc, 0, %1, vcc\n\t"
            : "=&v"(lo), "=&v"(hi)
            : "v"(init), "v"(m[4]), "s"(Stark252::p(7)), "v"(m[5]), "v"(a.v[4]), "v"(b.v[7]), "v"(a.v[5]), "v"(b.v[6]), "v"(a.v[6]), "v"(b.v[5]), "v"(a.v[7]), "v"(b.v[4])
            : "vcc");
    }
};

template <>
struct FusedCol<Stark252, 12, false> {
    __device__ static __forceinline__ void run(uint64_t &lo, uint32_t &hi, uint64_t init, const Fe<Stark252> &a, const Fe<Stark252> &b, const uint32_t (&m)[8]) {
        asm("v_mad_u64_u32 %0, vcc, %3, %4, %2\n\t"
            "v_mad_u64_u32 %0, vcc, %5, 17, %0\n\t"
            "v_mad_u64_u32 %0, vcc, %6, %7, %0\n\t"
            "v_addc_co_u32_e64 %1, vcc, 0, 0, vcc\n\t"
            "v_mad_u64_u32 %0, vcc, %8, %9, %0\n\t"
            "v_addc_co_u32_e32 %1, vcc, 0, %1, vcc\n\t"
            "v_mad_u64_u32 %0, vcc, %10, %11, %0\n\t"
            "v_addc_co_u32_e32 %1, vcc, 0, %1, vcc\n\t"
            : "=&v"(lo), "=&v"(hi)
            : "v"(init), "v"(m[5]), "s"(Stark252::p(7)), "v"(m[6]), "v"(a.v[5]), "v"(b.v[7]), "v"(a.v[6]), "v"(b.v[6]), "v"(a.v[7]), "v"(b.v[5])
            : "vcc");
    }
};

template <>
struct FusedCol<Stark252, 13, false> {
    __device__ static __forceinline__ void run(uint64_t &lo, uint32_t &hi, uint64_t init, const Fe<Stark252> &a, const Fe<Stark252> &b, const uint32_t (&m)[8]) {
        asm("v_mad_u64_u32 %0, vcc, %3, %4, %2\n\t"
            "v_mad_u64_u32 %0, vcc, %5, 17, %0\n\t"
            "v_mad_u64_u32 %0, vcc, %6, %7, %0\n\t"
            "v_addc_co_u32_e64 %1, vcc, 0, 0, vcc\n\t"
            "v_mad_u64_u32 %0, vcc, %8, %9, %0\n\t"
            "v_addc_co_u32_e32 %1, vcc, 0, %1, vcc\n\t"
            : "=&v"(lo), "=&v"(hi)
            : "v"(init), "v"(m[6]), "s"(Stark252::p(7)), "v"(m[7]), "v"(a.v[6]), "v"(b.v[7]), "v"(a.v[7]), "v"(b.v[6])
            : "vcc");
    }
};

template <>
struct FusedCol<Stark252, 14, false> {
    __device__ static __forceinline__ void run(uint64_t &lo, uint32_t &hi, uint64_t init, const Fe<Stark252> &a, const Fe<Stark252> &b, const uint32_t (&m)[8]) {
        asm("v_mad_u64_u32 %0, vcc, %2, %3, %1\n\t"
            "v_mad_u64_u32 %0, vcc, %4, %5, %0\n\t"
            : "=&v"(lo)
            : "v"(init), "v"(m[7]), "s"(Stark252::p(7)), "v"(a.v[7]), "v"(b.v[7])
            : "vcc");
        hi = 0;
    }
};

template <>
struct FusedCol<Stark252, 0, true> : FusedCol<Stark252, 0, false> {};

template <>
struct FusedCol<Stark252, 1, true> : FusedCol<Stark252, 1, false> {};

template <>
struct FusedCol<Stark252, 2, true> : FusedCol<Stark252, 2, false> {};

template <>
struct FusedCol<Stark252, 3, true> : FusedCol<Stark252, 3, false> {};

template <>
struct FusedCol<Stark252, 4, true> : FusedCol<Stark252, 4, false> {};

template <>
struct FusedCol<Stark252, 5, true> : FusedCol<Stark252, 5, false> {};

template <>
struct FusedCol<Stark252, 6, true> : FusedCol<Stark252, 6, false> {};

template <>
struct FusedCol<Stark252, 7, true> {
    __device__ static __forceinline__ void run(uint64_t &lo, uint32_t &hi, uint64_t init, const Fe<Stark252> &a, const Fe<Stark252> &b, const uint32_t (&m)[8]) {
        asm("v_mad_u64_u32 %0, vcc, %3, %4, %2\n\t"
            "v_mad_u64_u32 %0, vcc, %5, 17, %0\n\t"
            "v_mad_u64_u32 %0, vcc, %6, %7, %0\n\t"
            "v_mad_u64_u32 %0, vcc, %8, %9, %0\n\t"
            "v_addc_co_u32_e64 %1, vcc, 0, 0, vcc\n\t"
            "v_mad_u64_u32 %0, vcc, %10, %11, %0\n\t"
            "v_addc_co_u32_e32 %1, vcc, 0, %1, vcc\n\t"
            "v_mad_u64_u32 %0, vcc, %12, %13, %0\n\t"
            "v_addc_co_u32_e32 %1, vcc, 0, %1, vcc\n\t"
            "v_mad_u64_u32 %0, vcc, %14, %15, %0\n\t"
            "v_addc_co_u32_e32 %1, vcc, 0, %1, vcc\n\t"
            "v_mad_u64_u32 %0, vcc, %16, %17, %0\n\t"
            "v_addc_co_u32_e32 %1, vcc, 0, %1, vcc\n\t"
            "v_mad_u64_u32 %0, vcc, %18, %19, %0\n\t"
            "v_addc_co_u32_e32 %1, vcc, 0, %1, vcc\n\t"
            "v_mad_u64_u32 %0, vcc, %20, %21, %0\n\t"
            "v_addc_co_u32_e32 %1, vcc, 0, %1, vcc\n\t"
            : "=&v"(lo), "=&v"(hi)
            : "v"(init), "v"(m[0]), "s"(Stark252::p(7)), "v"(m[1]), "v"(a.v[7]), "v"(b.v[0]), "v"(a.v[0]), "v"(b.v[7]), "v"(a.v[1]), "v"(b.v[6]), "v"(a.v[2]), "v"(b.v[5]), "v"(a.v[3]), "v"(b.v[4]), "v"(a.v[4]), "v"(b.v[3]), "v"(a.v[5]), "v"(b.v[2]), "v"(a.v[6]), "v"(b.v[1])
            : "vcc");
    }
};

template <>
struct FusedCol<Stark252, 8, true> {
    __device__ static __forceinline__ void run(uint64_t &lo, uint32_t &hi, uint64_t init, const Fe<Stark252> &a, const Fe<Stark252> &b, const uint32_t (&m)[8]) {
        asm("v_mad_u64_u32 %0, vcc, %3, %4, %2\n\t"
            "v_mad_u64_u32 %0, vcc, %5, 17, %0\n\t"
            "v_mad_u64_u32 %0, vcc, %6, %7, %0\n\t"
            "v_mad_u64_u32 %0, vcc, %8, %9, %0\n\t"
            "v_addc_co_u32_e64 %1, vcc, 0, 0, vcc\n\t"
            "v_mad_u64_u32 %0, vcc, %10, %11, %0\n\t"
            "v_addc_co_u32_e32 %1, vcc, 0, %1, vcc\n\t"
            "v_mad_u64_u32 %0, vcc, %12, %13, %0\n\t"
            "v_addc_co_u32_e32 %1, vcc, 0, %1, vcc\n\t"
            "v_mad_u64_u32 %0, vcc, %14, %15, %0\n\t"
            "v_addc_co_u32_e32 %1, vcc, 0, %1, vcc\n\t"
            "v_mad_u64_u32 %0, vcc, %16, %17, %0\n\t"
            "v_addc_co_u32_e32 %1, vcc, 0, %1, vcc\n\t"
            "v_mad_u64_u32 %0, vcc, %18, %19, %0\n\t"
            "v_addc_co_u32_e32 %1, vcc, 0, %1, vcc\n\t"
            : "=&v"(lo), "=&v"(hi)
            : "v"(init), "v"(m[1]), "s"(Stark252::p(7)), "v"(m[2]), "v"(a.v[7]), "v"(b.v[1]), "v"(a.v[1]), "v"(b.v[7]), "v"(a.v[2]), "v"(b.v[6]), "v"(a.v[3]), "v"(b.v[5]), "v"(a.v[4]), "v"(b.v[4]), "v"(a.v[5]), "v"(b.v[3]), "v"(a.v[6]), "v"(b.v[2])
            : "vcc");
    }
};

template <>
struct FusedCol<Stark252, 9, true> {
    __device__ static __forceinline__ void run(uint64_t &lo, uint32_t &hi, uint64_t init, const Fe<Stark252> &a, const Fe<Stark252> &b, const uint32_t (&m)[8]) {
        asm("v_mad_u64_u32 %0, vcc, %3, %4, %2\n\t"
            "v_mad_u64_u32 %0, vcc, %5, 17, %0\n\t"
            "v_mad_u64_u32 %0, vcc, %6, %7, %0\n\t"
            "v_mad_u64_u32 %0, vcc, %8, %9, %0\n\t"
            "v_addc_co_u32_e64 %1, vcc, 0, 0, vcc\n\t"
            "v_mad_u64_u32 %0, vcc, %10, %11, %0\n\t"
            "v_addc_co_u32_e32 %1, vcc, 0, %1, vcc\n\t"
            "v_mad_u64_u32 %0, vcc, %12, %13, %0\n\t"
            "v_addc_co_u32_e32 %1, vcc, 0, %1, vcc\n\t"
            "v_mad_u64_u32 %0, vcc, %14, %15, %0\n\t"
            "v_addc_co_u32_e32 %1, vcc, 0, %1, vcc\n\t"
            "v_mad_u64_u32 %0, vcc, %16, %17, %0\n\t"
            "v_addc_co_u32_e32 %1, vcc, 0, %1, vcc\n\t"
            : "=&v"(lo), "=&v"(hi)
            : "v"(init), "v"(m[2]), "s"(Stark252::p(7)), "v"(m[3]), "v"(a.v[7]), "v"(b.v[2]), "v"(a.v[2]), "v"(b.v[7]), "v"(a.v[3]), "v"(b.v[6]), "v"(a.v[4]), "v"(b.v[5]), "v"(a.v[5]), "v"(b.v[4]), "v"(a.v[6]), "v"(b.v[3])
            : "vcc");
    }
};

template <>
struct FusedCol<Stark252, 10, true> {
    __device__ static __forceinline__ void run(uint64_t &lo, uint32_t &hi, uint64_t init, const Fe<Stark252> &a, const Fe<Stark252> &b, const uint32_t (&m)[8]) {
        asm("v_mad_u64_u32 %0, vcc, %3, %4, %2\n\t"
            "v_mad_u64_u32 %0, vcc, %5, 17, %0\n\t"
            "v_mad_u64_u32 %0, vcc, %6, %7, %0\n\t"
            "v_mad_u64_u32 %0, vcc, %8, %9, %0\n\t"
            "v_addc_co_u32_e64 %1, vcc, 0, 0, vcc\n\t"
            "v_mad_u64_u32 %0, vcc, %10, %11, %0\n\t"
            "v_addc_co_u32_e32 %1, vcc, 0, %1, vcc\n\t"
            "v_mad_u64_u32 %0, vcc, %12, %13, %0\n\t"
            "v_addc_co_u32_e32 %1, vcc, 0, %1, vcc\n\t"
            "v_mad_u64_u32 %0, vcc, %14, %15, %0\n\t"
            "v_addc_co_u32_e32 %1, vcc, 0, %1, vcc\n\t"
            : "=&v"(lo), "=&v"(hi)
            : "v"(init), "v"(m[3]), "s"(Stark252::p(7)), "v"(m[4]), "v"(a.v[7]), "v"(b.v[3]), "v"(a.v[3]), "v"(b.v[7]), "v"(a.v[4]), "v"(b.v[6]), "v"(a.v[5]), "v"(b.v[5]), "v"(a.v[6]), "v"(b.v[4])
            : "vcc");
    }
};

template <>
struct FusedCol<Stark252, 11, true> {
    __device__ static __forceinline__ void run(uint64_t &lo, uint32_t &hi, uint64_t init, const Fe<Stark252> &a, const Fe<Stark252> &b, const uint32_t (&m)[8]) {
        asm("v_mad_u64_u32 %0, vcc, %3, %4, %2\n\t"
            "v_mad_u64_u32 %0, vcc, %5, 17, %0\n\t"
            "v_mad_u64_u32 %0, vcc, %6, %7, %0\n\t"
            "v_mad_u64_u32 %0, vcc, %8, %9, %0\n\t"
            "v_addc_co_u32_e64 %1, vcc, 0, 0, vcc\n\t"
            "v_mad_u64_u32 %0, vcc, %10, %11, %0\n\t"
            "v_addc_co_u32_e32 %1, vcc, 0, %1, vcc\n\t"
            "v_mad_u64_u32 %0, vcc, %12, %13, %0\n\t"
            "v_addc_co_u32_e32 %1, vcc, 0, %1, vcc\n\t"
            : "=&v"(lo), "=&v"(hi)
            : "v"(init), "v"(m[4]), "s"(Stark252::p(7)), "v"(m[5]), "v"(a.v[7]), "v"(b.v[4]), "v"(a.v[4]), "v"(b.v[7]), "v"(a.v[5]), "v"(b.v[6]), "v"(a.v[6]), "v"(b.v[5])
            : "vcc");
    }
};

template <>
struct FusedCol<Stark252, 12, true> {
    __device__ static __forceinline__ void run(uint64_t &lo, uint32_t &hi, uint64_t init, const Fe<Stark252> &a, const Fe<Stark252> &b, const uint32_t (&m)[8]) {
        asm("v_mad_u64_u32 %0, vcc, %3, %4, %2\n\t"
            "v_mad_u64_u32 %0, vcc, %5, 17, %0\n\t"
            "v_mad_u64_u32 %0, vcc, %6, %7, %0\n\t"
            "v_mad_u64_u32 %0, vcc, %8, %9, %0\n\t"
            "v_addc_co_u32_e64 %1, vcc, 0, 0, vcc\n\t"
            "v_mad_u64_u32 %0, vcc, %10, %11, %0\n\t"
            "v_addc_co_u32_e32 %1, vcc, 0, %1, vcc\n\t"
            : "=&v"(lo), "=&v"(hi)
            : "v"(init), "v"(m[5]), "s"(Stark252::p(7)), "v"(m[6]), "v"(a.v[7]), "v"(b.v[5]), "v"(a.v[5]), "v"(b.v[7]), "v"(a.v[6]), "v"(b.v[6])
            : "vcc");
    }
};

template <>
struct FusedCol<Stark252, 13, true> {
    __device__ static __forceinline__ void run(uint64_t &lo, uint32_t &hi, uint64_t init, const Fe<Stark252> &a, const Fe<Stark252> &b, const uint32_t (&m)[8]) {
        asm("v_mad_u64_u32 %0, vcc, %3, %4, %2\n\t"
            "v_mad_u64_u32 %0, vcc, %5, 17, %0\n\t"
            "v_mad_u64_u32 %0, vcc, %6, %7, %0\n\t"
            "v_mad_u64_u32 %0, vcc, %8, %9, %0\n\t"
            "v_addc_co_u32_e64 %1, vcc, 0, 0, vcc\n\t"
            : "=&v"(lo), "=&v"(hi)
            : "v"(init), "v"(m[6]), "s"(Stark252::p(7)), "v"(m[7]), "v"(a.v[7]), "v"(b.v[6]), "v"(a.v[6]), "v"(b.v[7])
            : "vcc");
    }
};

template <>
struct FusedCol<Stark252, 14, true> : FusedCol<Stark252, 14, false> {};
```

### lambda_elliptic_curves_amd/csrc/ntt_kernels.cuh

```cuda
#pragma once
#include "field.cuh"

namespace lw {

constexpr int NTT_TILE_LOG = 11;
constexpr int NTT_TILE = 1 << NTT_TILE_LOG;
constexpr int NTT_THREADS = 512;
constexpr int NTT_KMAX = 2;
constexpr int NTT_WG_PER_CU = (160 * 1024) / (NTT_TILE * 32 + 8192) > 8 ? 8 : (160 * 1024) / (NTT_TILE * 32 + 8192);
constexpr int NTT_WAVES_PER_SIMD = (NTT_WG_PER_CU * NTT_THREADS / 256) > 8 ? 8 : (NTT_WG_PER_CU * NTT_THREADS / 256) < 1 ? 1 : (NTT_WG_PER_CU * NTT_THREADS / 256);
constexpr int NTT_LTW = 256;

struct NttPassParams {
    const uint4 *in;
    uint4 *out;
    const uint4 *tw;
    uint64_t in_batch_stride;
    uint64_t out_batch_stride;
    uint32_t L;
    uint32_t s0;
    uint32_t r;
    uint32_t logC;
    uint32_t nsteps;
    uint32_t k[8];
    const uint4 *cos_lo, *cos_hi;
    uint32_t cos_hbits;
    uint32_t cos_in;
    uint32_t cos_out;
    uint64_t in_mask;
    uint32_t lazy_in;
    uint32_t wave_sync;
    uint32_t scale;
    uint32_t sc[8];
};

__device__ __forceinline__ uint32_t bitrev_bits(uint32_t x, uint32_t bits) {
    return bits ? (__brev(x) >> (32 - bits)) : 0u;
}

template <class F>
__device__ __forceinline__ Fe<F> tw_load(const uint4 *tw, uint64_t g) {
    uint4 a = tw[2 * g], b = tw[2 * g + 1];
    Fe<F> r;
    r.v[0] = a.x; r.v[1] = a.y; r.v[2] = a.z; r.v[3] = a.w;
    r.v[4] = b.x; r.v[5] = b.y; r.v[6] = b.z; r.v[7] = b.w;
    return r;
}
template <class F>
__device__ __forceinline__ void tw_store(uint4 *tw, uint64_t g, const Fe<F> &x) {
    tw[2 * g] = make_uint4(x.v[0], x.v[1], x.v[2], x.v[3]);
    tw[2 * g + 1] = make_uint4(x.v[4], x.v[5], x.v[6], x.v[7]);
}

template <class F>
__device__ __forceinline__ Fe<F> unpack_mem(uint4 q0, uint4 q1) {
    Fe<F> r;
    r.v[6] = q0.x; r.v[7] = q0.y; r.v[4] = q0.z; r.v[5] = q0.w;
    r.v[2] = q1.x; r.v[3] = q1.y; r.v[0] = q1.z; r.v[1] = q1.w;
    return r;
}
template <class F>
__device__ __forceinline__ void pack_mem(const Fe<F> &a, uint4 &q0, uint4 &q1) {
    q0 = make_uint4(a.v[6], a.v[7], a.v[4], a.v[5]);
    q1 = make_uint4(a.v[2], a.v[3], a.v[0], a.v[1]);
}

template <bool WL>
__device__ __forceinline__ uint32_t lds_slot(uint32_t m, uint32_t c, uint32_t r, uint32_t logC) {
    if (!WL) return (m << logC) | c;
    const uint32_t sw = r >= 4 ? ((5u * ((m >> 4) & 3u)) ^ ((c & 7u) << 1)) : 0u;
    return (c << r) | (m ^ sw);
}
__device__ __forceinline__ void lds_wave_sync() {
    __builtin_amdgcn_fence(__ATOMIC_RELEASE, "wavefront");
    __builtin_amdgcn_wave_barrier();
    __builtin_amdgcn_fence(__ATOMIC_ACQUIRE, "wavefront");
}

template <class F, int K, bool LAST, bool EXTRA, bool WL, int FX = 0>
__device__ __forceinline__ void ntt_item(const NttPassParams &p, uint4 (*lds)[NTT_TILE], uint4 (*ltw)[NTT_LTW], const uint4 *gin,
                                         uint4 *gout, uint32_t w, uint32_t step, uint32_t t0, uint64_t base, uint32_t lgS,
                                         uint32_t hi_uniform, uint32_t hi_low, bool last_step, bool stage_tw) {
    constexpr int E = 1 << K;
    const uint32_t r = FX ? (uint32_t)FX : p.r, logC = FX ? (uint32_t)(NTT_TILE_LOG - FX) : p.logC, L = p.L;
    const uint32_t sh = r - t0 - K;
    uint32_t c, mr;
    if ((LAST && step == 0) || (WL && (LAST || step > 0))) {
        mr = w & ((1u << (r - K)) - 1);
        c = w >> (r - K);
    } else {
        c = w & ((1u << logC) - 1);
        mr = w >> logC;
    }
    const uint32_t m_low = mr & ((1u << sh) - 1);
    const uint32_t m_high = mr >> sh;
    const uint32_t mbase = (m_high << (sh + K)) | m_low;
    uint32_t hi_c = hi_uniform;
    uint64_t gbase = base;
    if (LAST) {
        hi_c = (bitrev_bits(c, logC) << (L - r - logC)) | hi_low;
        gbase = (uint64_t)hi_c << r;
    }

    uint4 tq0, tq1;
    const uint32_t ti = threadIdx.x;
    if (!LAST && !WL && stage_tw && ti + 1 < (1u << r)) {
        const uint32_t t = 31 - __clz(ti + 1), xg = ti + 1 - (1u << t);
        const uint64_t g = ((uint64_t)hi_uniform << t) | xg;
        tq0 = p.tw[2 * g];
        tq1 = p.tw[2 * g + 1];
    }

    Fe<F> x[E];
    if (step == 0) {
#pragma unroll
        for (int j = 0; j < E; j++) {
            const uint32_t m = mbase | ((uint32_t)j << sh);
            const uint64_t g = (LAST ? (gbase + m) : (gbase + ((uint64_t)m << lgS) + c)) & p.in_mask;
            x[j] = unpack_mem<F>(gin[2 * g], gin[2 * g + 1]);
        }
        if (EXTRA && p.cos_in) {
#pragma unroll
            for (int j = 0; j < E; j++) {
                const uint32_t m = mbase | ((uint32_t)j << sh);
                const uint64_t e = (LAST ? (gbase + m) : (gbase + ((uint64_t)m << lgS) + c)) & p.in_mask;
                Fe<F> pw = fe_mul<F>(tw_load<F>(p.cos_lo, e & ((1ull << p.cos_hbits) - 1)), tw_load<F>(p.cos_hi, e >> p.cos_hbits));
                x[j] = fe_mul<F>(x[j], pw);
            }
        }
    } else {
#pragma unroll
        for (int j = 0; j < E; j++) {
            const uint32_t idx = lds_slot<WL>(mbase | ((uint32_t)j << sh), c, r, logC);
            x[j] = unpack_mem<F>(lds[0][idx], lds[1][idx ^ (WL ? 1u : 0u)]);
        }
    }

    if (!LAST && !WL && stage_tw) {
        if (ti + 1 < (1u << r)) {
            ltw[0][ti] = tq0;
            ltw[1][ti] = tq1;
        }
        __syncthreads();
    }

    if (F::LAZY && step == 0 && p.lazy_in) {
#pragma unroll
        for (int j = 0; j < E / 2; j++) x[j] = fe_reduce_full(x[j]);
    }

    auto fetch_tw = [&](int q) -> Fe<F> {
        const int u = 31 - __builtin_clz(q + 1), jt = q + 1 - (1 << u);
        Fe<F> tw;
        if (LAST || WL) {
            const uint64_t gt = ((uint64_t)hi_c << (t0 + u)) | ((uint64_t)m_high << u);
            tw = tw_load<F>(p.tw, gt | (uint32_t)jt);
        } else {
            const uint32_t li = (1u << (t0 + u)) - 1 + ((m_high << u) | (uint32_t)jt);
            uint4 a = ltw[0][li], b = ltw[1][li];
            tw.v[0] = a.x; tw.v[1] = a.y; tw.v[2] = a.z; tw.v[3] = a.w;
            tw.v[4] = b.x; tw.v[5] = b.y; tw.v[6] = b.z; tw.v[7] = b.w;
        }
        return tw;
    };
    Fe<F> tw_next = fetch_tw(0);
#pragma unroll
    for (int q = 0; q < E - 1; q++) {
        const int u = 31 - __builtin_clz(q + 1), jt = q + 1 - (1 << u);
        const int half = 1 << (K - 1 - u);
        const Fe<F> tw = tw_next;
        if (q + 1 < E - 1) tw_next = fetch_tw(q + 1);
        const bool unit = (jt == 0) && (hi_c == 0) && (m_high == 0);
#pragma unroll
        for (int jl = 0; jl < half; jl++) {
            const int j = (jt << (K - u)) | jl;
            if (F::LAZY) {
                Fe<F> wb = unit ? fe_reduce_full(x[j + half]) : fe_mul_lazy<F>(tw, x[j + half]);
                Fe<F> a = x[j];
                x[j] = fe_add_raw<F>(a, wb);
                x[j + half] = fe_add2p_sub_raw<F>(a, wb);
            } else {
                Fe<F> wb = unit ? x[j + half] : fe_mul<F>(tw, x[j + half]);
                Fe<F> a = x[j];
                x[j] = fe_add<F>(a, wb);
                x[j + half] = fe_sub<F>(a, wb);
            }
            __builtin_amdgcn_sched_barrier(0);
        }
    }

    if (EXTRA && LAST && last_step && p.cos_out) {
#pragma unroll
        for (int j = 0; j < E; j++) {
            const uint32_t m = mbase | ((uint32_t)j << sh);
            const uint64_t i_nat = ((uint64_t)bitrev_bits(m, r) << (L - r)) + ((uint64_t)blockIdx.x << logC) + c;
            Fe<F> pw = fe_mul<F>(tw_load<F>(p.cos_lo, i_nat & ((1ull << p.cos_hbits) - 1)), tw_load<F>(p.cos_hi, i_nat >> p.cos_hbits));
            if (F::LAZY) x[j] = fe_cond_sub_kp<F, 0>(fe_mul_lazy<F>(pw, x[j]));
            else x[j] = fe_mul<F>(x[j], pw);
        }
    } else if (EXTRA && last_step && p.scale) {
        Fe<F> sc;
#pragma unroll
        for (int i = 0; i < 8; i++) sc.v[i] = p.sc[i];
#pragma unroll
        for (int j = 0; j < E; j++) {
            if (F::LAZY) x[j] = fe_cond_sub_kp<F, 0>(fe_mul_lazy<F>(sc, x[j]));
            else x[j] = fe_mul<F>(x[j], sc);
        }
    } else if (F::LAZY && LAST && last_step) {
#pragma unroll
        for (int j = 0; j < E; j++) x[j] = fe_reduce_full(x[j]);
    }

    if (!LAST && last_step) {
#pragma unroll
        for (int j = 0; j < E; j++) {
            const uint32_t m = mbase | ((uint32_t)j << sh);
            const uint64_t g = gbase + ((uint64_t)m << lgS) + c;
            uint4 q0, q1;
            pack_mem<F>(x[j], q0, q1);
            gout[2 * g] = q0;
            gout[2 * g + 1] = q1;
        }
        return;
    }
#pragma unroll
    for (int j = 0; j < E; j++) {
        const uint32_t idx = lds_slot<WL>(mbase | ((uint32_t)j << sh), c, r, logC);
        uint4 q0, q1;
        pack_mem<F>(x[j], q0, q1);
        lds[0][idx] = q0;
        lds[1][idx ^ (WL ? 1u : 0u)] = q1;
    }
}

template <class F, bool LAST, bool EXTRA, bool WL, int FX = 0>
__global__ __launch_bounds__(NTT_THREADS, NTT_WAVES_PER_SIMD) void ntt_pass_kernel(NttPassParams p) {
    __shared__ uint4 lds[2][NTT_TILE];
    __shared__ uint4 ltw[LAST ? 1 : 2][LAST ? 1 : NTT_LTW];
    const uint32_t tid = threadIdx.x;
    static_assert(!FX || (NTT_TILE == 2048 && NTT_THREADS == 512 && (FX == 8 || FX == 7 || FX == 6)), "FX: 2^8 x 8, 2^7 x 16 or 2^6 x 32 rows x columns");
    const uint32_t r = FX ? (uint32_t)FX : p.r, logC = FX ? (uint32_t)(NTT_TILE_LOG - FX) : p.logC, L = p.L;
    const uint32_t tile_log = r + logC;
    const uint4 *gin = p.in + 2 * (uint64_t)blockIdx.y * p.in_batch_stride;
    uint4 *gout = p.out + 2 * (uint64_t)blockIdx.y * p.out_batch_stride;
    const uint32_t b = blockIdx.x;

    uint64_t base = 0;
    uint32_t lgS = 0, hi_uniform = 0, hi_low = 0;
    if (!LAST) {
        lgS = L - p.s0 - r;
        const uint32_t lo_bits = lgS - logC;
        const uint32_t lo_blk = b & ((1u << lo_bits) - 1);
        hi_uniform = b >> lo_bits;
        base = ((uint64_t)hi_uniform << (L - p.s0)) + ((uint64_t)lo_blk << logC);
    } else {
        hi_low = bitrev_bits(b, L - r - logC);
    }

    const bool stage_inside = FX ? (!LAST && !WL)
                                 : (!LAST && !WL && (1u << (tile_log - p.k[0])) >= (uint32_t)NTT_THREADS && (1u << r) <= (uint32_t)NTT_THREADS);
    if (!LAST && !WL && !stage_inside) {
        for (uint32_t i = tid; i + 1 < (1u << r); i += NTT_THREADS) {
            const uint32_t t = 31 - __clz(i + 1), x = i + 1 - (1u << t);
            const uint64_t g = ((uint64_t)hi_uniform << t) | x;
            ltw[0][i] = p.tw[2 * g];
            ltw[1][i] = p.tw[2 * g + 1];
        }
        __syncthreads();
    }
    if constexpr (FX) {
#define LW_FX_STEP(S)                                                                                                                  \
    do {                                                                                                                                \
        if (S) {                                                                                                                        \
            if (WL && ((p.wave_sync >> (S)) & 1u)) lds_wave_sync();                                                                     \
            else __syncthreads();                                                                                                       \
        }                                                                                                                               \
        ntt_item<F, 2, LAST, EXTRA, WL, FX>(p, lds, (uint4 (*)[NTT_LTW])ltw, gin, gout, tid, (S), 2u * (S), base, lgS, hi_uniform, hi_low,    \
                                            2 * ((S) + 1) == FX, stage_inside && (S) == 0);                                             \
    } while (0)
        LW_FX_STEP(0u);
        LW_FX_STEP(1u);
        LW_FX_STEP(2u);
        if constexpr (FX == 8) LW_FX_STEP(3u);
        if constexpr (FX == 7) {
            __syncthreads();
            ntt_item<F, 1, LAST, EXTRA, WL, FX>(p, lds, (uint4 (*)[NTT_LTW])ltw, gin, gout, tid, 3u, 6u, base, lgS, hi_uniform, hi_low, true, false);
            ntt_item<F, 1, LAST, EXTRA, WL, FX>(p, lds, (uint4 (*)[NTT_LTW])ltw, gin, gout, tid + NTT_THREADS, 3u, 6u, base, lgS, hi_uniform, hi_low, true, false);
        }
#undef LW_FX_STEP
    } else {
    uint32_t t0 = 0;
    for (uint32_t step = 0; step < p.nsteps; step++) {
        const uint32_t k = p.k[step];
        const uint32_t nitems = 1u << (tile_log - k);
        const bool last_step = (step + 1 == p.nsteps);
        if (step) {
            if (WL && ((p.wave_sync >> step) & 1u)) lds_wave_sync();
            else __syncthreads();
        }
        for (uint32_t w = tid; w < nitems; w += NTT_THREADS) {
            if (NTT_KMAX >= 3 && k == 3) ntt_item<F, (NTT_KMAX >= 3 ? 3 : 1), LAST, EXTRA, WL>(p, lds, (uint4 (*)[NTT_LTW])ltw, gin, gout, w, step, t0, base, lgS, hi_uniform, hi_low, last_step, stage_inside && step == 0 && w == tid);
            else if (k == 2) ntt_item<F, 2, LAST, EXTRA, WL>(p, lds, (uint4 (*)[NTT_LTW])ltw, gin, gout, w, step, t0, base, lgS, hi_uniform, hi_low, last_step, stage_inside && step == 0 && w == tid);
            else ntt_item<F, 1, LAST, EXTRA, WL>(p, lds, (uint4 (*)[NTT_LTW])ltw, gin, gout, w, step, t0, base, lgS, hi_uniform, hi_low, last_step, stage_inside && step == 0 && w == tid);
        }
        t0 += k;
    }
    }
    if constexpr (!LAST) return;
    __syncthreads();

    auto write_one = [&](uint32_t f) {
        const uint32_t e = f >> 1, plane = f & 1;
        const uint32_t c = e & ((1u << logC) - 1);
        const uint32_t m = e >> logC;
        const uint64_t g = ((uint64_t)bitrev_bits(m, r) << (L - r)) + ((uint64_t)b << logC) + c;
        gout[2 * g + plane] = lds[plane][lds_slot<WL>(m, c, r, logC) ^ (WL ? plane : 0u)];
    };
    if constexpr (FX) {
#pragma unroll
        for (int q = 0; q < 2 * NTT_TILE / NTT_THREADS; q++) write_one(tid + (uint32_t)q * NTT_THREADS);
    } else {
        const uint32_t total = 2u << tile_log;
        for (uint32_t f = tid; f < total; f += NTT_THREADS) write_one(f);
    }
}

template <class F>
__global__ void twiddle_fill_kernel(uint4 *tw, const uint4 *lo, const uint4 *hi, uint32_t bits, uint32_t hbits,
                                    uint64_t count) {
    uint64_t g = (uint64_t)blockIdx.x * blockDim.x + threadIdx.x;
    if (g >= count) return;
    uint32_t e = bitrev_bits((uint32_t)g, bits);
    Fe<F> a = tw_load<F>(lo, e & ((1u << hbits) - 1));
    Fe<F> b = tw_load<F>(hi, e >> hbits);
    tw_store<F>(tw, g, fe_mul<F>(a, b));
}

struct FeWords8 {
    uint32_t w[8];
};
template <class F>
__global__ void power_tables_kernel(uint4 *lo, uint4 *hi, FeWords8 base, uint32_t hbits, uint64_t hi_count, FeWords8 scale, int has_scale) {
    const uint64_t t = (uint64_t)blockIdx.x * blockDim.x + threadIdx.x;
    const uint64_t lo_count = 1ull << hbits;
    if (t >= lo_count + hi_count) return;
    const bool is_lo = t < lo_count;
    const uint64_t e = is_lo ? t : ((t - lo_count) << hbits);
    Fe<F> b, r = Fe<F>::one();
#pragma unroll
    for (int k = 0; k < 8; k++) b.v[k] = base.w[k];
    for (int bit = 63 - (e ? __clzll((long long)e) : 63); bit >= 0; bit--) {
        r = fe_sqr<F>(r);
        if ((e >> bit) & 1) r = fe_mul<F>(r, b);
    }
    if (!is_lo && has_scale) {
        Fe<F> sc;
#pragma unroll
        for (int k = 0; k < 8; k++) sc.v[k] = scale.w[k];
        r = fe_mul<F>(r, sc);
    }
    if (is_lo) tw_store<F>(lo, t, r);
    else tw_store<F>(hi, t - lo_count, r);
}

}
```

Before: 13.44 billion.

## Add register-resident FX tile path with scalar-operand twiddle multiplies and one LDS plane

Adds Montgomery multiply column chains that take the wave-uniform operand (twiddle) from SGPRs, so uniform twiddles stop occupying VGPRs. Non-last FX passes get a new tile routine that keeps four elements per thread in registers and exchanges them through a single LDS plane in two halves, which halves LDS use. It also raises the launch-bounds waves-per-SIMD target from 4 to 6 when prefetch is disabled. The aim is higher occupancy and fewer LDS round trips, at the cost of extra barriers per exchange and possible register spills if the tighter register budget is exceeded.

Result: faster. 13.81 billion, median of 6 (+2.8%).

```diff
diff --git a/lambda_elliptic_curves_amd/csrc/field.cuh b/lambda_elliptic_curves_amd/csrc/field.cuh
--- a/lambda_elliptic_curves_amd/csrc/field.cuh
+++ b/lambda_elliptic_curves_amd/csrc/field.cuh
@@ -398,6 +398,8 @@
 };
 template <class F, int K, bool A_LT_P>
 struct FusedCol;
+template <class F, int K>
+struct FusedColS;
 #include "mac_chains.inc"
 
 template <class F, int LO, int HI>
@@ -456,7 +458,7 @@
         : "v"(t), "v"(w1)
         : "vcc");
 }
-template <class F, int K, bool A_LT_P>
+template <class F, int K, bool A_LT_P, bool A_SGPR = false>
 __device__ __forceinline__ void fips_fused(uint64_t init, const Fe<F> &a, const Fe<F> &b, uint32_t (&m)[F::N], uint32_t (&t)[F::N]) {
     constexpr int N = F::N;
     static_assert(F::p(0) == 1u && F::INV == 0xffffffffu, "fused columns need a unit low limb of the modulus");
@@ -465,23 +467,25 @@
     } else {
         uint64_t lo;
         uint32_t hi;
-        FusedCol<F, K, A_LT_P>::run(lo, hi, init, a, b, m);
+        static_assert(A_LT_P || !A_SGPR, "the scalar-operand columns exist for a < p only");
+        if constexpr (A_SGPR) FusedColS<F, K>::run(lo, hi, init, a, b, m);
+        else FusedCol<F, K, A_LT_P>::run(lo, hi, init, a, b, m);
         if constexpr (K < N) {
             uint32_t mid, top;
             if constexpr (K == 0) lw_redc_unit0(m[0], mid, top, (uint32_t)lo, (uint32_t)(lo >> 32));
             else lw_redc_unit(m[K], mid, top, (uint32_t)lo, (uint32_t)(lo >> 32), hi);
-            fips_fused<F, K + 1, A_LT_P>(((uint64_t)top << 32) | mid, a, b, m, t);
+            fips_fused<F, K + 1, A_LT_P, A_SGPR>(((uint64_t)top << 32) | mid, a, b, m, t);
         } else {
             t[K - N] = (uint32_t)lo;
-            fips_fused<F, K + 1, A_LT_P>((lo >> 32) | ((uint64_t)hi << 32), a, b, m, t);
-        }
-    }
-}
-template <class F, bool A_LT_P = false>
+            fips_fused<F, K + 1, A_LT_P, A_SGPR>((lo >> 32) | ((uint64_t)hi << 32), a, b, m, t);
+        }
+    }
+}
+template <class F, bool A_LT_P = false, bool A_SGPR = false>
 __device__ __forceinline__ void fips_product(const Fe<F> &a, const Fe<F> &b, uint32_t (&t)[F::N]) {
     uint32_t m[F::N];
     if constexpr (lw_fused_columns<F>::value) {
-        fips_fused<F, 0, A_LT_P>(0ull, a, b, m, t);
+        fips_fused<F, 0, A_LT_P, A_SGPR>(0ull, a, b, m, t);
     } else {
         const Fe<F> *const pa[1] = {&a}, *const pb[1] = {&b};
         fips_col<F, 1, 0>(0ull, pa, pb, m, t);
@@ -599,6 +603,20 @@
     constexpr int N = F::N;
     uint32_t t[N];
     fips_product<F, true>(a, b, t);
+    Fe<F> r;
+#pragma unroll
+    for (int i = 0; i < N; i++) r.v[i] = t[i];
+    return r;
+#else
+    return fe_mul_portable<F>(a, b);
+#endif
+}
+template <class F>
+LW_HD Fe<F> fe_mul_lazy_uniform(const Fe<F> &a, const Fe<F> &b) {
+#if defined(__HIP_DEVICE_COMPILE__)
+    constexpr int N = F::N;
+    uint32_t t[N];
+    fips_product<F, true, lw_fused_columns<F>::value>(a, b, t);
     Fe<F> r;
 #pragma unroll
     for (int i = 0; i < N; i++) r.v[i] = t[i];
diff --git a/lambda_elliptic_curves_amd/csrc/mac_chains.inc b/lambda_elliptic_curves_amd/csrc/mac_chains.inc
--- a/lambda_elliptic_curves_amd/csrc/mac_chains.inc
+++ b/lambda_elliptic_curves_amd/csrc/mac_chains.inc
@@ -662,3 +662,274 @@
 
 template <>
 struct FusedCol<Stark252, 14, true> : FusedCol<Stark252, 14, false> {};
+
+
+template <>
+struct FusedColS<Stark252, 0> {
+    __device__ static __forceinline__ void run(uint64_t &lo, uint32_t &hi, uint64_t init, const Fe<Stark252> &a, const Fe<Stark252> &b, const uint32_t (&m)[8]) {
+        asm("v_mad_u64_u32 %0, vcc, %1, %2, 0\n\t"
+            : "=v"(lo)
+            : "s"(a.v[0]), "v"(b.v[0])
+            : "vcc");
+        hi = 0;
+    }
+};
+
+template <>
+struct FusedColS<Stark252, 1> {
+    __device__ static __forceinline__ void run(uint64_t &lo, uint32_t &hi, uint64_t init, const Fe<Stark252> &a, const Fe<Stark252> &b, const uint32_t (&m)[8]) {
+        asm("v_mad_u64_u32 %0, vcc, %3, %4, %2\n\t"
+            "v_mad_u64_u32 %0, vcc, %5, %6, %0\n\t"
+            "v_addc_co_u32_e64 %1, vcc, 0, 0, vcc\n\t"
+            : "=&v"(lo), "=&v"(hi)
+            : "v"(init), "s"(a.v[0]), "v"(b.v[1]), "s"(a.v[1]), "v"(b.v[0])
+            : "vcc");
+    }
+};
+
+template <>
+struct FusedColS<Stark252, 2> {
+    __device__ static __forceinline__ void run(uint64_t &lo, uint32_t &hi, uint64_t init, const Fe<Stark252> &a, const Fe<Stark252> &b, const uint32_t (&m)[8]) {
+        asm("v_mad_u64_u32 %0, vcc, %3, %4, %2\n\t"
+            "v_mad_u64_u32 %0, vcc, %5, %6, %0\n\t"
+            "v_addc_co_u32_e64 %1, vcc, 0, 0, vcc\n\t"
+            "v_mad_u64_u32 %0, vcc, %7, %8, %0\n\t"
+            "v_addc_co_u32_e32 %1, vcc, 0, %1, vcc\n\t"
+            : "=&v"(lo), "=&v"(hi)
+            : "v"(init), "s"(a.v[0]), "v"(b.v[2]), "s"(a.v[1]), "v"(b.v[1]), "s"(a.v[2]), "v"(b.v[0])
+            : "vcc");
+    }
+};
+
+template <>
+struct FusedColS<Stark252, 3> {
+    __device__ static __forceinline__ void run(uint64_t &lo, uint32_t &hi, uint64_t init, const Fe<Stark252> &a, const Fe<Stark252> &b, const uint32_t (&m)[8]) {
+        asm("v_mad_u64_u32 %0, vcc, %3, %4, %2\n\t"
+            "v_addc_co_u32_e64 %1, vcc, 0, 0, vcc\n\t"
+            "v_mad_u64_u32 %0, vcc, %5, %6, %0\n\t"
+            "v_addc_co_u32_e32 %1, vcc, 0, %1, vcc\n\t"
+            "v_mad_u64_u32 %0, vcc, %7, %8, %0\n\t"
+            "v_addc_co_u32_e32 %1, vcc, 0, %1, vcc\n\t"
+            "v_mad_u64_u32 %0, vcc, %9, %10, %0\n\t"
+            "v_addc_co_u32_e32 %1, vcc, 0, %1, vcc\n\t"
+            : "=&v"(lo), "=&v"(hi)
+            : "v"(init), "s"(a.v[0]), "v"(b.v[3]), "s"(a.v[1]), "v"(b.v[2]), "s"(a.v[2]), "v"(b.v[1]), "s"(a.v[3]), "v"(b.v[0])
+            : "vcc");
+    }
+};
+
+template <>
+struct FusedColS<Stark252, 4> {
+    __device__ static __forceinline__ void run(uint64_t &lo, uint32_t &hi, uint64_t init, const Fe<Stark252> &a, const Fe<Stark252> &b, const uint32_t (&m)[8]) {
+        asm("v_mad_u64_u32 %0, vcc, %3, %4, %2\n\t"
+            "v_addc_co_u32_e64 %1, vcc, 0, 0, vcc\n\t"
+            "v_mad_u64_u32 %0, vcc, %5, %6, %0\n\t"
+            "v_addc_co_u32_e32 %1, vcc, 0, %1, vcc\n\t"
+            "v_mad_u64_u32 %0, vcc, %7, %8, %0\n\t"
+            "v_addc_co_u32_e32 %1, vcc, 0, %1, vcc\n\t"
+            "v_mad_u64_u32 %0, vcc, %9, %10, %0\n\t"
+            "v_addc_co_u32_e32 %1, vcc, 0, %1, vcc\n\t"
+            "v_mad_u64_u32 %0, vcc, %11, %12, %0\n\t"
+            "v_addc_co_u32_e32 %1, vcc, 0, %1, vcc\n\t"
+            : "=&v"(lo), "=&v"(hi)
+            : "v"(init), "s"(a.v[0]), "v"(b.v[4]), "s"(a.v[1]), "v"(b.v[3]), "s"(a.v[2]), "v"(b.v[2]), "s"(a.v[3]), "v"(b.v[1]), "s"(a.v[4]), "v"(b.v[0])
+            : "vcc");
+    }
+};
+
+template <>
+struct FusedColS<Stark252, 5> {
+    __device__ static __forceinline__ void run(uint64_t &lo, uint32_t &hi, uint64_t init, const Fe<Stark252> &a, const Fe<Stark252> &b, const uint32_t (&m)[8]) {
+        asm("v_mad_u64_u32 %0, vcc, %3, %4, %2\n\t"
+            "v_addc_co_u32_e64 %1, vcc, 0, 0, vcc\n\t"
+            "v_mad_u64_u32 %0, vcc, %5, %6, %0\n\t"
+            "v_addc_co_u32_e32 %1, vcc, 0, %1, vcc\n\t"
+            "v_mad_u64_u32 %0, vcc, %7, %8, %0\n\t"
+            "v_addc_co_u32_e32 %1, vcc, 0, %1, vcc\n\t"
+            "v_mad_u64_u32 %0, vcc, %9, %10, %0\n\t"
+            "v_addc_co_u32_e32 %1, vcc, 0, %1, vcc\n\t"
+            "v_mad_u64_u32 %0, vcc, %11, %12, %0\n\t"
+            "v_addc_co_u32_e32 %1, vcc, 0, %1, vcc\n\t"
+            "v_mad_u64_u32 %0, vcc, %13, %14, %0\n\t"
+            "v_addc_co_u32_e32 %1, vcc, 0, %1, vcc\n\t"
+            : "=&v"(lo), "=&v"(hi)
+            : "v"(init), "s"(a.v[0]), "v"(b.v[5]), "s"(a.v[1]), "v"(b.v[4]), "s"(a.v[2]), "v"(b.v[3]), "s"(a.v[3]), "v"(b.v[2]), "s"(a.v[4]), "v"(b.v[1]), "s"(a.v[5]), "v"(b.v[0])
+            : "vcc");
+    }
+};
+
+template <>
+struct FusedColS<Stark252, 6> {
+    __device__ static __forceinline__ void run(uint64_t &lo, uint32_t &hi, uint64_t init, const Fe<Stark252> &a, const Fe<Stark252> &b, const uint32_t (&m)[8]) {
+        asm("v_mad_u64_u32 %0, vcc, %3, 17, %2\n\t"
+            "v_mad_u64_u32 %0, vcc, %4, %5, %0\n\t"
+            "v_addc_co_u32_e64 %1, vcc, 0, 0, vcc\n\t"
+            "v_mad_u64_u32 %0, vcc, %6, %7, %0\n\t"
+            "v_addc_co_u32_e32 %1, vcc, 0, %1, vcc\n\t"
+            "v_mad_u64_u32 %0, vcc, %8, %9, %0\n\t"
+            "v_addc_co_u32_e32 %1, vcc, 0, %1, vcc\n\t"
+            "v_mad_u64_u32 %0, vcc, %10, %11, %0\n\t"
+            "v_addc_co_u32_e32 %1, vcc, 0, %1, vcc\n\t"
+            "v_mad_u64_u32 %0, vcc, %12, %13, %0\n\t"
+            "v_addc_co_u32_e32 %1, vcc, 0, %1, vcc\n\t"
+            "v_mad_u64_u32 %0, vcc, %14, %15, %0\n\t"
+            "v_addc_co_u32_e32 %1, vcc, 0, %1, vcc\n\t"
+            "v_mad_u64_u32 %0, vcc, %16, %17, %0\n\t"
+            "v_addc_co_u32_e32 %1, vcc, 0, %1, vcc\n\t"
+            : "=&v"(lo), "=&v"(hi)
+            : "v"(init), "v"(m[0]), "s"(a.v[0]), "v"(b.v[6]), "s"(a.v[1]), "v"(b.v[5]), "s"(a.v[2]), "v"(b.v[4]), "s"(a.v[3]), "v"(b.v[3]), "s"(a.v[4]), "v"(b.v[2]), "s"(a.v[5]), "v"(b.v[1]), "s"(a.v[6]), "v"(b.v[0])
+            : "vcc");
+    }
+};
+
+template <>
+struct FusedColS<Stark252, 7> {
+    __device__ static __forceinline__ void run(uint64_t &lo, uint32_t &hi, uint64_t init, const Fe<Stark252> &a, const Fe<Stark252> &b, const uint32_t (&m)[8]) {
+        asm("v_mad_u64_u32 %0, vcc, %3, %4, %2\n\t"
+            "v_mad_u64_u32 %0, vcc, %5, 17, %0\n\t"
+            "v_mad_u64_u32 %0, vcc, %6, %7, %0\n\t"
+            "v_mad_u64_u32 %0, vcc, %8, %9, %0\n\t"
+            "v_addc_co_u32_e64 %1, vcc, 0, 0, vcc\n\t"
+            "v_mad_u64_u32 %0, vcc, %10, %11, %0\n\t"
+            "v_addc_co_u32_e32 %1, vcc, 0, %1, vcc\n\t"
+            "v_mad_u64_u32 %0, vcc, %12, %13, %0\n\t"
+            "v_addc_co_u32_e32 %1, vcc, 0, %1, vcc\n\t"
+            "v_mad_u64_u32 %0, vcc, %14, %15, %0\n\t"
+            "v_addc_co_u32_e32 %1, vcc, 0, %1, vcc\n\t"
+            "v_mad_u64_u32 %0, vcc, %16, %17, %0\n\t"
+            "v_addc_co_u32_e32 %1, vcc, 0, %1, vcc\n\t"
+            "v_mad_u64_u32 %0, vcc, %18, %19, %0\n\t"
+            "v_addc_co_u32_e32 %1, vcc, 0, %1, vcc\n\t"
+            "v_mad_u64_u32 %0, vcc, %20, %21, %0\n\t"
+            "v_addc_co_u32_e32 %1, vcc, 0, %1, vcc\n\t"
+            : "=&v"(lo), "=&v"(hi)
+            : "v"(init), "v"(m[0]), "s"(Stark252::p(7)), "v"(m[1]), "s"(a.v[7]), "v"(b.v[0]), "s"(a.v[0]), "v"(b.v[7]), "s"(a.v[1]), "v"(b.v[6]), "s"(a.v[2]), "v"(b.v[5]), "s"(a.v[3]), "v"(b.v[4]), "s"(a.v[4]), "v"(b.v[3]), "s"(a.v[5]), "v"(b.v[2]), "s"(a.v[6]), "v"(b.v[1])
+            : "vcc");
+    }
+};
+
+template <>
+struct FusedColS<Stark252, 8> {
+    __device__ static __forceinline__ void run(uint64_t &lo, uint32_t &hi, uint64_t init, const Fe<Stark252> &a, const Fe<Stark252> &b, const uint32_t (&m)[8]) {
+        asm("v_mad_u64_u32 %0, vcc, %3, %4, %2\n\t"
+            "v_mad_u64_u32 %0, vcc, %5, 17, %0\n\t"
+            "v_mad_u64_u32 %0, vcc, %6, %7, %0\n\t"
+            "v_mad_u64_u32 %0, vcc, %8, %9, %0\n\t"
+            "v_addc_co_u32_e64 %1, vcc, 0, 0, vcc\n\t"
+            "v_mad_u64_u32 %0, vcc, %10, %11, %0\n\t"
+            "v_addc_co_u32_e32 %1, vcc, 0, %1, vcc\n\t"
+            "v_mad_u64_u32 %0, vcc, %12, %13, %0\n\t"
+            "v_addc_co_u32_e32 %1, vcc, 0, %1, vcc\n\t"
+            "v_mad_u64_u32 %0, vcc, %14, %15, %0\n\t"
+            "v_addc_co_u32_e32 %1, vcc, 0, %1, vcc\n\t"
+            "v_mad_u64_u32 %0, vcc, %16, %17, %0\n\t"
+            "v_addc_co_u32_e32 %1, vcc, 0, %1, vcc\n\t"
+            "v_mad_u64_u32 %0, vcc, %18, %19, %0\n\t"
+            "v_addc_co_u32_e32 %1, vcc, 0, %1, vcc\n\t"
+            : "=&v"(lo), "=&v"(hi)
+            : "v"(init), "v"(m[1]), "s"(Stark252::p(7)), "v"(m[2]), "s"(a.v[7]), "v"(b.v[1]), "s"(a.v[1]), "v"(b.v[7]), "s"(a.v[2]), "v"(b.v[6]), "s"(a.v[3]), "v"(b.v[5]), "s"(a.v[4]), "v"(b.v[4]), "s"(a.v[5]), "v"(b.v[3]), "s"(a.v[6]), "v"(b.v[2])
+            : "vcc");
+    }
+};
+
+template <>
+struct FusedColS<Stark252, 9> {
+    __device__ static __forceinline__ void run(uint64_t &lo, uint32_t &hi, uint64_t init, const Fe<Stark252> &a, const Fe<Stark252> &b, const uint32_t (&m)[8]) {
+        asm("v_mad_u64_u32 %0, vcc, %3, %4, %2\n\t"
+            "v_mad_u64_u32 %0, vcc, %5, 17, %0\n\t"
+            "v_mad_u64_u32 %0, vcc, %6, %7, %0\n\t"
+            "v_mad_u64_u32 %0, vcc, %8, %9, %0\n\t"
+            "v_addc_co_u32_e64 %1, vcc, 0, 0, vcc\n\t"
+            "v_mad_u64_u32 %0, vcc, %10, %11, %0\n\t"
+            "v_addc_co_u32_e32 %1, vcc, 0, %1, vcc\n\t"
+            "v_mad_u64_u32 %0, vcc, %12, %13, %0\n\t"
+            "v_addc_co_u32_e32 %1, vcc, 0, %1, vcc\n\t"
+            "v_mad_u64_u32 %0, vcc, %14, %15, %0\n\t"
+            "v_addc_co_u32_e32 %1, vcc, 0, %1, vcc\n\t"
+            "v_mad_u64_u32 %0, vcc, %16, %17, %0\n\t"
+            "v_addc_co_u32_e32 %1, vcc, 0, %1, vcc\n\t"
+            : "=&v"(lo), "=&v"(hi)
+            : "v"(init), "v"(m[2]), "s"(Stark252::p(7)), "v"(m[3]), "s"(a.v[7]), "v"(b.v[2]), "s"(a.v[2]), "v"(b.v[7]), "s"(a.v[3]), "v"(b.v[6]), "s"(a.v[4]), "v"(b.v[5]), "s"(a.v[5]), "v"(b.v[4]), "s"(a.v[6]), "v"(b.v[3])
+            : "vcc");
+    }
+};
+
+template <>
+struct FusedColS<Stark252, 10> {
+    __device__ static __forceinline__ void run(uint64_t &lo, uint32_t &hi, uint64_t init, const Fe<Stark252> &a, const Fe<Stark252> &b, const uint32_t (&m)[8]) {
+        asm("v_mad_u64_u32 %0, vcc, %3, %4, %2\n\t"
+            "v_mad_u64_u32 %0, vcc, %5, 17, %0\n\t"
+            "v_mad_u64_u32 %0, vcc, %6, %7, %0\n\t"
+            "v_mad_u64_u32 %0, vcc, %8, %9, %0\n\t"
+            "v_addc_co_u32_e64 %1, vcc, 0, 0, vcc\n\t"
+            "v_mad_u64_u32 %0, vcc, %10, %11, %0\n\t"
+            "v_addc_co_u32_e32 %1, vcc, 0, %1, vcc\n\t"
+            "v_mad_u64_u32 %0, vcc, %12, %13, %0\n\t"
+            "v_addc_co_u32_e32 %1, vcc, 0, %1, vcc\n\t"
+            "v_mad_u64_u32 %0, vcc, %14, %15, %0\n\t"
+            "v_addc_co_u32_e32 %1, vcc, 0, %1, vcc\n\t"
+            : "=&v"(lo), "=&v"(hi)
+            : "v"(init), "v"(m[3]), "s"(Stark252::p(7)), "v"(m[4]), "s"(a.v[7]), "v"(b.v[3]), "s"(a.v[3]), "v"(b.v[7]), "s"(a.v[4]), "v"(b.v[6]), "s"(a.v[5]), "v"(b.v[5]), "s"(a.v[6]), "v"(b.v[4])
+            : "vcc");
+    }
+};
+
+template <>
+struct FusedColS<Stark252, 11> {
+    __device__ static __forceinline__ void run(uint64_t &lo, uint32_t &hi, uint64_t init, const Fe<Stark252> &a, const Fe<Stark252> &b, const uint32_t (&m)[8]) {
+        asm("v_mad_u64_u32 %0, vcc, %3, %4, %2\n\t"
+            "v_mad_u64_u32 %0, vcc, %5, 17, %0\n\t"
+            "v_mad_u64_u32 %0, vcc, %6, %7, %0\n\t"
+            "v_mad_u64_u32 %0, vcc, %8, %9, %0\n\t"
+            "v_addc_co_u32_e64 %1, vcc, 0, 0, vcc\n\t"
+            "v_mad_u64_u32 %0, vcc, %10, %11, %0\n\t"
+            "v_addc_co_u32_e32 %1, vcc, 0, %1, vcc\n\t"
+            "v_mad_u64_u32 %0, vcc, %12, %13, %0\n\t"
+            "v_addc_co_u32_e32 %1, vcc, 0, %1, vcc\n\t"
+            : "=&v"(lo), "=&v"(hi)
+            : "v"(init), "v"(m[4]), "s"(Stark252::p(7)), "v"(m[5]), "s"(a.v[7]), "v"(b.v[4]), "s"(a.v[4]), "v"(b.v[7]), "s"(a.v[5]), "v"(b.v[6]), "s"(a.v[6]), "v"(b.v[5])
+            : "vcc");
+    }
+};
+
+template <>
+struct FusedColS<Stark252, 12> {
+    __device__ static __forceinline__ void run(uint64_t &lo, uint32_t &hi, uint64_t init, const Fe<Stark252> &a, const Fe<Stark252> &b, const uint32_t (&m)[8]) {
+        asm("v_mad_u64_u32 %0, vcc, %3, %4, %2\n\t"
+            "v_mad_u64_u32 %0, vcc, %5, 17, %0\n\t"
+            "v_mad_u64_u32 %0, vcc, %6, %7, %0\n\t"
+            "v_mad_u64_u32 %0, vcc, %8, %9, %0\n\t"
+            "v_addc_co_u32_e64 %1, vcc, 0, 0, vcc\n\t"
+            "v_mad_u64_u32 %0, vcc, %10, %11, %0\n\t"
+            "v_addc_co_u32_e32 %1, vcc, 0, %1, vcc\n\t"
+            : "=&v"(lo), "=&v"(hi)
+            : "v"(init), "v"(m[5]), "s"(Stark252::p(7)), "v"(m[6]), "s"(a.v[7]), "v"(b.v[5]), "s"(a.v[5]), "v"(b.v[7]), "s"(a.v[6]), "v"(b.v[6])
+            : "vcc");
+    }
+};
+
+template <>
+struct FusedColS<Stark252, 13> {
+    __device__ static __forceinline__ void run(uint64_t &lo, uint32_t &hi, uint64_t init, const Fe<Stark252> &a, const Fe<Stark252> &b, const uint32_t (&m)[8]) {
+        asm("v_mad_u64_u32 %0, vcc, %3, %4, %2\n\t"
+            "v_mad_u64_u32 %0, vcc, %5, 17, %0\n\t"
+            "v_mad_u64_u32 %0, vcc, %6, %7, %0\n\t"
+            "v_mad_u64_u32 %0, vcc, %8, %9, %0\n\t"
+            "v_addc_co_u32_e64 %1, vcc, 0, 0, vcc\n\t"
+            : "=&v"(lo), "=&v"(hi)
+            : "v"(init), "v"(m[6]), "s"(Stark252::p(7)), "v"(m[7]), "s"(a.v[7]), "v"(b.v[6]), "s"(a.v[6]), "v"(b.v[7])
+            : "vcc");
+    }
+};
+
+template <>
+struct FusedColS<Stark252, 14> {
+    __device__ static __forceinline__ void run(uint64_t &lo, uint32_t &hi, uint64_t init, const Fe<Stark252> &a, const Fe<Stark252> &b, const uint32_t (&m)[8]) {
+        asm("v_mad_u64_u32 %0, vcc, %2, %3, %1\n\t"
+            "v_mad_u64_u32 %0, vcc, %4, %5, %0\n\t"
+            : "=&v"(lo)
+            : "v"(init), "v"(m[7]), "s"(Stark252::p(7)), "s"(a.v[7]), "v"(b.v[7])
+            : "vcc");
+        hi = 0;
+    }
+};
diff --git a/lambda_elliptic_curves_amd/csrc/ntt_kernels.cuh b/lambda_elliptic_curves_amd/csrc/ntt_kernels.cuh
--- a/lambda_elliptic_curves_amd/csrc/ntt_kernels.cuh
+++ b/lambda_elliptic_curves_amd/csrc/ntt_kernels.cuh
@@ -7,8 +7,6 @@
 constexpr int NTT_TILE = 1 << NTT_TILE_LOG;
 constexpr int NTT_THREADS = 512;
 constexpr int NTT_KMAX = 2;
-constexpr int NTT_WG_PER_CU = (160 * 1024) / (NTT_TILE * 32 + 8192) > 8 ? 8 : (160 * 1024) / (NTT_TILE * 32 + 8192);
-constexpr int NTT_WAVES_PER_SIMD = (NTT_WG_PER_CU * NTT_THREADS / 256) > 8 ? 8 : (NTT_WG_PER_CU * NTT_THREADS / 256) < 1 ? 1 : (NTT_WG_PER_CU * NTT_THREADS / 256);
 constexpr int NTT_LTW = 256;
 
 struct NttPassParams {
@@ -47,6 +45,15 @@
     return r;
 }
 template <class F>
+__device__ __forceinline__ Fe<F> tw_load_uniform(const uint4 *tw, uint64_t g) {
+    typedef const __attribute__((address_space(4))) uint32_t *const_words;
+    const_words w = (const_words)(uintptr_t)(tw + 2 * g);
+    Fe<F> r;
+#pragma unroll
+    for (int i = 0; i < 8; i++) r.v[i] = w[i];
+    return r;
+}
+template <class F>
 __device__ __forceinline__ void tw_store(uint4 *tw, uint64_t g, const Fe<F> &x) {
     tw[2 * g] = make_uint4(x.v[0], x.v[1], x.v[2], x.v[3]);
     tw[2 * g + 1] = make_uint4(x.v[4], x.v[5], x.v[6], x.v[7]);
@@ -77,105 +84,124 @@
     __builtin_amdgcn_fence(__ATOMIC_ACQUIRE, "wavefront");
 }
 
-template <class F, int K, bool LAST, bool EXTRA, bool WL, int FX = 0>
-__device__ __forceinline__ void ntt_item(const NttPassParams &p, uint4 (*lds)[NTT_TILE], uint4 (*ltw)[NTT_LTW], const uint4 *gin,
-                                         uint4 *gout, uint32_t w, uint32_t step, uint32_t t0, uint64_t base, uint32_t lgS,
-                                         uint32_t hi_uniform, uint32_t hi_low, bool last_step, bool stage_tw) {
-    constexpr int E = 1 << K;
+struct NttItemGeo {
+    uint32_t c, mbase, m_high, sh;
+    uint32_t hi_c;
+    uint64_t gbase;
+};
+template <int K, bool LAST, bool WL, int FX>
+__device__ __forceinline__ NttItemGeo ntt_item_geo(const NttPassParams &p, uint32_t w, uint32_t step, uint32_t t0, uint64_t base,
+                                                   uint32_t hi_uniform, uint32_t hi_low) {
     const uint32_t r = FX ? (uint32_t)FX : p.r, logC = FX ? (uint32_t)(NTT_TILE_LOG - FX) : p.logC, L = p.L;
-    const uint32_t sh = r - t0 - K;
-    uint32_t c, mr;
+    NttItemGeo g;
+    g.sh = r - t0 - K;
+    uint32_t mr;
     if ((LAST && step == 0) || (WL && (LAST || step > 0))) {
         mr = w & ((1u << (r - K)) - 1);
-        c = w >> (r - K);
-    } else {
-        c = w & ((1u << logC) - 1);
+        g.c = w >> (r - K);
+    } else {
+        g.c = w & ((1u << logC) - 1);
         mr = w >> logC;
     }
-    const uint32_t m_low = mr & ((1u << sh) - 1);
-    const uint32_t m_high = mr >> sh;
-    const uint32_t mbase = (m_high << (sh + K)) | m_low;
-    uint32_t hi_c = hi_uniform;
-    uint64_t gbase = base;
+    const uint32_t m_low = mr & ((1u << g.sh) - 1);
+    g.m_high = mr >> g.sh;
+    g.mbase = (g.m_high << (g.sh + K)) | m_low;
+    g.hi_c = hi_uniform;
+    g.gbase = base;
     if (LAST) {
-        hi_c = (bitrev_bits(c, logC) << (L - r - logC)) | hi_low;
-        gbase = (uint64_t)hi_c << r;
-    }
-
-    uint4 tq0, tq1;
+        g.hi_c = (bitrev_bits(g.c, logC) << (L - r - logC)) | hi_low;
+        g.gbase = (uint64_t)g.hi_c << r;
+    }
+    return g;
+}
+
+__device__ __forceinline__ void ntt_tw_stage_load(const NttPassParams &p, uint32_t r, uint32_t hi_uniform, uint4 &tq0, uint4 &tq1) {
     const uint32_t ti = threadIdx.x;
-    if (!LAST && !WL && stage_tw && ti + 1 < (1u << r)) {
+    if (ti + 1 < (1u << r)) {
         const uint32_t t = 31 - __clz(ti + 1), xg = ti + 1 - (1u << t);
         const uint64_t g = ((uint64_t)hi_uniform << t) | xg;
         tq0 = p.tw[2 * g];
         tq1 = p.tw[2 * g + 1];
     }
-
-    Fe<F> x[E];
-    if (step == 0) {
+}
+__device__ __forceinline__ void ntt_tw_stage_store(uint4 (*ltw)[NTT_LTW], uint32_t r, const uint4 &tq0, const uint4 &tq1) {
+    const uint32_t ti = threadIdx.x;
+    if (ti + 1 < (1u << r)) {
+        ltw[0][ti] = tq0;
+        ltw[1][ti] = tq1;
+    }
+}
+
+template <class F, int K, bool LAST, bool EXTRA>
+__device__ __forceinline__ void ntt_load_global(const NttPassParams &p, const NttItemGeo &g, const uint4 *gin, uint32_t lgS, Fe<F> *x) {
+    constexpr int E = 1 << K;
+#pragma unroll
+    for (int j = 0; j < E; j++) {
+        const uint32_t m = g.mbase | ((uint32_t)j << g.sh);
+        const uint64_t e = (LAST ? (g.gbase + m) : (g.gbase + ((uint64_t)m << lgS) + g.c)) & p.in_mask;
+        x[j] = unpack_mem<F>(gin[2 * e], gin[2 * e + 1]);
+    }
+    if (EXTRA && p.cos_in) {
 #pragma unroll
         for (int j = 0; j < E; j++) {
-            const uint32_t m = mbase | ((uint32_t)j << sh);
-            const uint64_t g = (LAST ? (gbase + m) : (gbase + ((uint64_t)m << lgS) + c)) & p.in_mask;
-            x[j] = unpack_mem<F>(gin[2 * g], gin[2 * g + 1]);
-        }
-        if (EXTRA && p.cos_in) {
-#pragma unroll
-            for (int j = 0; j < E; j++) {
-                const uint32_t m = mbase | ((uint32_t)j << sh);
-                const uint64_t e = (LAST ? (gbase + m) : (gbase + ((uint64_t)m << lgS) + c)) & p.in_mask;
-                Fe<F> pw = fe_mul<F>(tw_load<F>(p.cos_lo, e & ((1ull << p.cos_hbits) - 1)), tw_load<F>(p.cos_hi, e >> p.cos_hbits));
-                x[j] = fe_mul<F>(x[j], pw);
-            }
-        }
-    } else {
-#pragma unroll
-        for (int j = 0; j < E; j++) {
-            const uint32_t idx = lds_slot<WL>(mbase | ((uint32_t)j << sh), c, r, logC);
-            x[j] = unpack_mem<F>(lds[0][idx], lds[1][idx ^ (WL ? 1u : 0u)]);
-        }
-    }
-
-    if (!LAST && !WL && stage_tw) {
-        if (ti + 1 < (1u << r)) {
-            ltw[0][ti] = tq0;
-            ltw[1][ti] = tq1;
-        }
-        __syncthreads();
-    }
-
-    if (F::LAZY && step == 0 && p.lazy_in) {
+            const uint32_t m = g.mbase | ((uint32_t)j << g.sh);
+            const uint64_t e = (LAST ? (g.gbase + m) : (g.gbase + ((uint64_t)m << lgS) + g.c)) & p.in_mask;
+            Fe<F> pw = fe_mul<F>(tw_load<F>(p.cos_lo, e & ((1ull << p.cos_hbits) - 1)), tw_load<F>(p.cos_hi, e >> p.cos_hbits));
+            x[j] = fe_mul<F>(x[j], pw);
+        }
+    }
+}
+
+template <class F, bool LAST, bool WL>
+__device__ __forceinline__ Fe<F> ntt_fetch_tw(const NttPassParams &p, const NttItemGeo &g, uint4 (*ltw)[NTT_LTW], uint32_t t0, int q) {
+    const int u = 31 - __builtin_clz(q + 1), jt = q + 1 - (1 << u);
+    Fe<F> tw;
+    if (LAST || WL) {
+        const uint64_t gt = ((uint64_t)g.hi_c << (t0 + u)) | ((uint64_t)g.m_high << u);
+        tw = tw_load<F>(p.tw, gt | (uint32_t)jt);
+    } else {
+        const uint32_t li = (1u << (t0 + u)) - 1 + ((g.m_high << u) | (uint32_t)jt);
+        uint4 a = ltw[0][li], b = ltw[1][li];
+        tw.v[0] = a.x; tw.v[1] = a.y; tw.v[2] = a.z; tw.v[3] = a.w;
+        tw.v[4] = b.x; tw.v[5] = b.y; tw.v[6] = b.z; tw.v[7] = b.w;
+    }
+    return tw;
+}
+
+template <class F, int K, bool LAST, bool WL, bool PF, bool UNI = false>
+__device__ __forceinline__ void ntt_butterflies(const NttPassParams &p, const NttItemGeo &g, uint4 (*ltw)[NTT_LTW], uint32_t t0, bool first,
+                                                Fe<F> *x) {
+    constexpr int E = 1 << K;
+    static_assert(!UNI || (!LAST && !WL), "wave-uniform twiddles: plain non-last passes only");
+    const uint32_t m_high = UNI ? (uint32_t)__builtin_amdgcn_readfirstlane((int)g.m_high) : g.m_high;
+    if (F::LAZY && first && p.lazy_in) {
 #pragma unroll
         for (int j = 0; j < E / 2; j++) x[j] = fe_reduce_full(x[j]);
     }
 
-    auto fetch_tw = [&](int q) -> Fe<F> {
-        const int u = 31 - __builtin_clz(q + 1), jt = q + 1 - (1 << u);
-        Fe<F> tw;
-        if (LAST || WL) {
-            const uint64_t gt = ((uint64_t)hi_c << (t0 + u)) | ((uint64_t)m_high << u);
-            tw = tw_load<F>(p.tw, gt | (uint32_t)jt);
-        } else {
-            const uint32_t li = (1u << (t0 + u)) - 1 + ((m_high << u) | (uint32_t)jt);
-            uint4 a = ltw[0][li], b = ltw[1][li];
-            tw.v[0] = a.x; tw.v[1] = a.y; tw.v[2] = a.z; tw.v[3] = a.w;
-            tw.v[4] = b.x; tw.v[5] = b.y; tw.v[6] = b.z; tw.v[7] = b.w;
-        }
-        return tw;
-    };
-    Fe<F> tw_next = fetch_tw(0);
+    auto fetch_tw = [&](int q) -> Fe<F> { return ntt_fetch_tw<F, LAST, WL>(p, g, ltw, t0, q); };
+    Fe<F> tw_next, tw_uni[E - 1];
+    if (UNI) {
+#pragma unroll
+        for (int q = 0; q < E - 1; q++) {
+            const int u = 31 - __builtin_clz(q + 1), jt = q + 1 - (1 << u);
+            tw_uni[q] = tw_load_uniform<F>(p.tw, ((uint64_t)g.hi_c << (t0 + u)) | ((uint64_t)m_high << u) | (uint32_t)jt);
+        }
+    } else if (PF) {
+        tw_next = fetch_tw(0);
+    }
 #pragma unroll
     for (int q = 0; q < E - 1; q++) {
         const int u = 31 - __builtin_clz(q + 1), jt = q + 1 - (1 << u);
         const int half = 1 << (K - 1 - u);
-        const Fe<F> tw = tw_next;
-        if (q + 1 < E - 1) tw_next = fetch_tw(q + 1);
-        const bool unit = (jt == 0) && (hi_c == 0) && (m_high == 0);
+        const Fe<F> tw = UNI ? tw_uni[q] : PF ? tw_next : fetch_tw(q);
+        if (!UNI && PF && q + 1 < E - 1) tw_next = fetch_tw(q + 1);
+        const bool unit = (jt == 0) && (g.hi_c == 0) && (m_high == 0);
 #pragma unroll
         for (int jl = 0; jl < half; jl++) {
             const int j = (jt << (K - u)) | jl;
             if (F::LAZY) {
-                Fe<F> wb = unit ? fe_reduce_full(x[j + half]) : fe_mul_lazy<F>(tw, x[j + half]);
+                Fe<F> wb = unit ? fe_reduce_full(x[j + half]) : UNI ? fe_mul_lazy_uniform<F>(tw, x[j + half]) : fe_mul_lazy<F>(tw, x[j + half]);
                 Fe<F> a = x[j];
                 x[j] = fe_add_raw<F>(a, wb);
                 x[j + half] = fe_add2p_sub_raw<F>(a, wb);
@@ -188,17 +214,22 @@
             __builtin_amdgcn_sched_barrier(0);
         }
     }
-
-    if (EXTRA && LAST && last_step && p.cos_out) {
+}
+
+template <class F, int K, bool LAST, bool EXTRA, int FX>
+__device__ __forceinline__ void ntt_finish(const NttPassParams &p, const NttItemGeo &g, Fe<F> *x) {
+    constexpr int E = 1 << K;
+    const uint32_t r = FX ? (uint32_t)FX : p.r, logC = FX ? (uint32_t)(NTT_TILE_LOG - FX) : p.logC, L = p.L;
+    if (EXTRA && LAST && p.cos_out) {
 #pragma unroll
         for (int j = 0; j < E; j++) {
-            const uint32_t m = mbase | ((uint32_t)j << sh);
-            const uint64_t i_nat = ((uint64_t)bitrev_bits(m, r) << (L - r)) + ((uint64_t)blockIdx.x << logC) + c;
+            const uint32_t m = g.mbase | ((uint32_t)j << g.sh);
+            const uint64_t i_nat = ((uint64_t)bitrev_bits(m, r) << (L - r)) + ((uint64_t)blockIdx.x << logC) + g.c;
             Fe<F> pw = fe_mul<F>(tw_load<F>(p.cos_lo, i_nat & ((1ull << p.cos_hbits) - 1)), tw_load<F>(p.cos_hi, i_nat >> p.cos_hbits));
             if (F::LAZY) x[j] = fe_cond_sub_kp<F, 0>(fe_mul_lazy<F>(pw, x[j]));
             else x[j] = fe_mul<F>(x[j], pw);
         }
-    } else if (EXTRA && last_step && p.scale) {
+    } else if (EXTRA && p.scale) {
         Fe<F> sc;
 #pragma unroll
         for (int i = 0; i < 8; i++) sc.v[i] = p.sc[i];
@@ -207,39 +238,141 @@
             if (F::LAZY) x[j] = fe_cond_sub_kp<F, 0>(fe_mul_lazy<F>(sc, x[j]));
             else x[j] = fe_mul<F>(x[j], sc);
         }
-    } else if (F::LAZY && LAST && last_step) {
+    } else if (F::LAZY && LAST) {
 #pragma unroll
         for (int j = 0; j < E; j++) x[j] = fe_reduce_full(x[j]);
     }
-
-    if (!LAST && last_step) {
-#pragma unroll
-        for (int j = 0; j < E; j++) {
-            const uint32_t m = mbase | ((uint32_t)j << sh);
-            const uint64_t g = gbase + ((uint64_t)m << lgS) + c;
-            uint4 q0, q1;
-            pack_mem<F>(x[j], q0, q1);
-            gout[2 * g] = q0;
-            gout[2 * g + 1] = q1;
-        }
-        return;
-    }
-#pragma unroll
-    for (int j = 0; j < E; j++) {
-        const uint32_t idx = lds_slot<WL>(mbase | ((uint32_t)j << sh), c, r, logC);
+}
+
+template <class F, int K>
+__device__ __forceinline__ void ntt_store_global(const NttItemGeo &g, uint4 *gout, uint32_t lgS, const Fe<F> *x) {
+#pragma unroll
+    for (int j = 0; j < (1 << K); j++) {
+        const uint32_t m = g.mbase | ((uint32_t)j << g.sh);
+        const uint64_t e = g.gbase + ((uint64_t)m << lgS) + g.c;
         uint4 q0, q1;
         pack_mem<F>(x[j], q0, q1);
-        lds[0][idx] = q0;
-        lds[1][idx ^ (WL ? 1u : 0u)] = q1;
+        gout[2 * e] = q0;
+        gout[2 * e + 1] = q1;
+    }
+}
+
+template <class F, int K, bool LAST, bool EXTRA, bool WL, int FX = 0>
+__device__ __forceinline__ void ntt_item(const NttPassParams &p, uint4 (*lds)[NTT_TILE], uint4 (*ltw)[NTT_LTW], const uint4 *gin,
+                                         uint4 *gout, uint32_t w, uint32_t step, uint32_t t0, uint64_t base, uint32_t lgS,
+                                         uint32_t hi_uniform, uint32_t hi_low, bool last_step, bool stage_tw) {
+    constexpr int E = 1 << K;
+    const uint32_t r = FX ? (uint32_t)FX : p.r, logC = FX ? (uint32_t)(NTT_TILE_LOG - FX) : p.logC;
+    const NttItemGeo g = ntt_item_geo<K, LAST, WL, FX>(p, w, step, t0, base, hi_uniform, hi_low);
+    uint4 tq0, tq1;
+    if (!LAST && !WL && stage_tw) ntt_tw_stage_load(p, r, hi_uniform, tq0, tq1);
+    Fe<F> x[E];
+    if (step == 0) {
+        ntt_load_global<F, K, LAST, EXTRA>(p, g, gin, lgS, x);
+    } else {
+#pragma unroll
+        for (int j = 0; j < E; j++) {
+            const uint32_t idx = lds_slot<WL>(g.mbase | ((uint32_t)j << g.sh), g.c, r, logC);
+            x[j] = unpack_mem<F>(lds[0][idx], lds[1][idx ^ (WL ? 1u : 0u)]);
+        }
+    }
+    if (!LAST && !WL && stage_tw) {
+        ntt_tw_stage_store(ltw, r, tq0, tq1);
+        __syncthreads();
+    }
+    ntt_butterflies<F, K, LAST, WL, true>(p, g, ltw, t0, step == 0, x);
+    if (last_step) ntt_finish<F, K, LAST, EXTRA, FX>(p, g, x);
+    if (!LAST && last_step) {
+        ntt_store_global<F, K>(g, gout, lgS, x);
+        return;
+    }
+#pragma unroll
+    for (int j = 0; j < E; j++) {
+        const uint32_t idx = lds_slot<WL>(g.mbase | ((uint32_t)j << g.sh), g.c, r, logC);
+        pack_mem<F>(x[j], lds[0][idx], lds[1][idx ^ (WL ? 1u : 0u)]);
+    }
+}
+
+template <bool LAST, int FX>
+constexpr bool ntt_one_plane() { return FX && !LAST; }
+template <class F, bool LAST, bool EXTRA, int FX>
+constexpr int ntt_waves_per_simd() { return ntt_one_plane<LAST, FX>() && F::LAZY && !EXTRA ? 6 : 4; }
+
+template <class F>
+__device__ __forceinline__ void ntt_exchange(uint4 *lds, const uint32_t (&so)[4], const uint32_t (&si)[4], Fe<F> *x) {
+    uint4 o0[4], o1[4], n0[4];
+#pragma unroll
+    for (int j = 0; j < 4; j++) pack_mem<F>(x[j], o0[j], o1[j]);
+#pragma unroll
+    for (int j = 0; j < 4; j++) lds[so[j]] = o0[j];
+    __syncthreads();
+#pragma unroll
+    for (int j = 0; j < 4; j++) n0[j] = lds[si[j]];
+    __syncthreads();
+#pragma unroll
+    for (int j = 0; j < 4; j++) lds[so[j]] = o1[j];
+    __syncthreads();
+#pragma unroll
+    for (int j = 0; j < 4; j++) x[j] = unpack_mem<F>(n0[j], lds[si[j]]);
+}
+
+template <int K, int FX>
+__device__ __forceinline__ void ntt_item_slots(const NttItemGeo &g, uint32_t *s) {
+#pragma unroll
+    for (int j = 0; j < (1 << K); j++) s[j] = lds_slot<false>(g.mbase | ((uint32_t)j << g.sh), g.c, FX, NTT_TILE_LOG - FX);
+}
+
+template <class F, bool EXTRA, int FX>
+__device__ __forceinline__ void ntt_tile_fx(const NttPassParams &p, uint4 *lds, uint4 (*ltw)[NTT_LTW], const uint4 *gin, uint4 *gout,
+                                            uint64_t base, uint32_t lgS, uint32_t hi_uniform) {
+    constexpr bool PF = ntt_waves_per_simd<F, false, EXTRA, FX>() < 6;
+    static_assert(NTT_TILE_LOG - NTT_KMAX == 9 && NTT_THREADS == 512, "wave-uniform twiddles of steps 0 and 1 assume 512 radix-4 items");
+    const uint32_t tid = threadIdx.x;
+    Fe<F> x[4];
+    uint32_t so[4], si[4];
+
+    NttItemGeo g = ntt_item_geo<2, false, false, FX>(p, tid, 0u, 0u, base, hi_uniform, 0u);
+    uint4 tq0, tq1;
+    ntt_tw_stage_load(p, FX, hi_uniform, tq0, tq1);
+    ntt_load_global<F, 2, false, EXTRA>(p, g, gin, lgS, x);
+    ntt_tw_stage_store(ltw, FX, tq0, tq1);
+    ntt_butterflies<F, 2, false, false, PF, true>(p, g, ltw, 0u, true, x);
+    ntt_item_slots<2, FX>(g, so);
+#pragma unroll
+    for (uint32_t s = 1; s < FX / 2; s++) {
+        g = ntt_item_geo<2, false, false, FX>(p, tid, s, 2 * s, base, hi_uniform, 0u);
+        ntt_item_slots<2, FX>(g, si);
+        ntt_exchange<F>(lds, so, si, x);
+        if (s == 1) ntt_butterflies<F, 2, false, false, PF, true>(p, g, ltw, 2 * s, false, x);
+        else ntt_butterflies<F, 2, false, false, PF>(p, g, ltw, 2 * s, false, x);
+#pragma unroll
+        for (int j = 0; j < 4; j++) so[j] = si[j];
+    }
+    if constexpr (FX % 2) {
+        const NttItemGeo ga = ntt_item_geo<1, false, false, FX>(p, tid, FX / 2, FX - 1, base, hi_uniform, 0u);
+        const NttItemGeo gb = ntt_item_geo<1, false, false, FX>(p, tid + NTT_THREADS, FX / 2, FX - 1, base, hi_uniform, 0u);
+        ntt_item_slots<1, FX>(ga, si);
+        ntt_item_slots<1, FX>(gb, si + 2);
+        ntt_exchange<F>(lds, so, si, x);
+        ntt_butterflies<F, 1, false, false, PF>(p, ga, ltw, FX - 1, false, x);
+        ntt_butterflies<F, 1, false, false, PF>(p, gb, ltw, FX - 1, false, x + 2);
+        ntt_finish<F, 1, false, EXTRA, FX>(p, ga, x);
+        ntt_finish<F, 1, false, EXTRA, FX>(p, gb, x + 2);
+        ntt_store_global<F, 1>(ga, gout, lgS, x);
+        ntt_store_global<F, 1>(gb, gout, lgS, x + 2);
+    } else {
+        ntt_finish<F, 2, false, EXTRA, FX>(p, g, x);
+        ntt_store_global<F, 2>(g, gout, lgS, x);
     }
 }
 
 template <class F, bool LAST, bool EXTRA, bool WL, int FX = 0>
-__global__ __launch_bounds__(NTT_THREADS, NTT_WAVES_PER_SIMD) void ntt_pass_kernel(NttPassParams p) {
-    __shared__ uint4 lds[2][NTT_TILE];
+__global__ __launch_bounds__(NTT_THREADS, (ntt_waves_per_simd<F, LAST, EXTRA, FX>())) void ntt_pass_kernel(NttPassParams p) {
+    __shared__ uint4 lds[ntt_one_plane<LAST, FX>() ? 1 : 2][NTT_TILE];
     __shared__ uint4 ltw[LAST ? 1 : 2][LAST ? 1 : NTT_LTW];
     const uint32_t tid = threadIdx.x;
     static_assert(!FX || (NTT_TILE == 2048 && NTT_THREADS == 512 && (FX == 8 || FX == 7 || FX == 6)), "FX: 2^8 x 8, 2^7 x 16 or 2^6 x 32 rows x columns");
+    static_assert(!WL || LAST, "the column layout is the last pass's");
     const uint32_t r = FX ? (uint32_t)FX : p.r, logC = FX ? (uint32_t)(NTT_TILE_LOG - FX) : p.logC, L = p.L;
     const uint32_t tile_log = r + logC;
     const uint4 *gin = p.in + 2 * (uint64_t)blockIdx.y * p.in_batch_stride;
@@ -258,17 +391,9 @@
         hi_low = bitrev_bits(b, L - r - logC);
     }
 
-    const bool stage_inside = FX ? (!LAST && !WL)
-                                 : (!LAST && !WL && (1u << (tile_log - p.k[0])) >= (uint32_t)NTT_THREADS && (1u << r) <= (uint32_t)NTT_THREADS);
-    if (!LAST && !WL && !stage_inside) {
-        for (uint32_t i = tid; i + 1 < (1u << r); i += NTT_THREADS) {
-            const uint32_t t = 31 - __clz(i + 1), x = i + 1 - (1u << t);
-            const uint64_t g = ((uint64_t)hi_uniform << t) | x;
-            ltw[0][i] = p.tw[2 * g];
-            ltw[1][i] = p.tw[2 * g + 1];
-        }
-        __syncthreads();
-    }
+    if constexpr (ntt_one_plane<LAST, FX>()) {
+        ntt_tile_fx<F, EXTRA, FX>(p, lds[0], (uint4 (*)[NTT_LTW])ltw, gin, gout, base, lgS, hi_uniform);
+    } else {
     if constexpr (FX) {
 #define LW_FX_STEP(S)                                                                                                                  \
     do {                                                                                                                                \
@@ -277,7 +402,7 @@
             else __syncthreads();                                                                                                       \
         }                                                                                                                               \
         ntt_item<F, 2, LAST, EXTRA, WL, FX>(p, lds, (uint4 (*)[NTT_LTW])ltw, gin, gout, tid, (S), 2u * (S), base, lgS, hi_uniform, hi_low,    \
-                                            2 * ((S) + 1) == FX, stage_inside && (S) == 0);                                             \
+                                            2 * ((S) + 1) == FX, false);                                                                \
     } while (0)
         LW_FX_STEP(0u);
         LW_FX_STEP(1u);
@@ -290,6 +415,16 @@
         }
 #undef LW_FX_STEP
     } else {
+    const bool stage_inside = !LAST && !WL && (1u << (tile_log - p.k[0])) >= (uint32_t)NTT_THREADS && (1u << r) <= (uint32_t)NTT_THREADS;
+    if (!LAST && !WL && !stage_inside) {
+        for (uint32_t i = tid; i + 1 < (1u << r); i += NTT_THREADS) {
+            const uint32_t t = 31 - __clz(i + 1), x = i + 1 - (1u << t);
+            const uint64_t g = ((uint64_t)hi_uniform << t) | x;
+            ltw[0][i] = p.tw[2 * g];
+            ltw[1][i] = p.tw[2 * g + 1];
+        }
+        __syncthreads();
+    }
     uint32_t t0 = 0;
     for (uint32_t step = 0; step < p.nsteps; step++) {
         const uint32_t k = p.k[step];
@@ -324,6 +459,7 @@
         const uint32_t total = 2u << tile_log;
         for (uint32_t f = tid; f < total; f += NTT_THREADS) write_one(f);
     }
+    }
 }
 
 template <class F>
```
